# NVIDIA/CUDALibrarySamples

Hardware: AMD Instinct MI355X
Metric: contraction GFLOP/s, fp32 einsum abcd,dcbe->ae (higher is better)
Workload: dtype f32

## Files before the change

### cudalibrarysamples_amd/csrc/host/api.cpp

```cpp
#include <algorithm>
#include <cmath>
#include <cstdio>
#include <cstdlib>
#include <cstring>
#include <new>
#include <optional>
#include <sstream>

#include <hip/hip_runtime.h>

#include "internal.hpp"

using namespace ctamd;

static const cutensorComputeDescriptor kCompute[6] = {
    {0, CUTENSOR_COMPUTE_16F}, {1, CUTENSOR_COMPUTE_16BF}, {2, CUTENSOR_COMPUTE_TF32},
    {3, CUTENSOR_COMPUTE_3XTF32}, {4, CUTENSOR_COMPUTE_32F}, {5, CUTENSOR_COMPUTE_64F}};
extern "C" {
const cutensorComputeDescriptor_t CUTENSOR_COMPUTE_DESC_16F    = &kCompute[0];
const cutensorComputeDescriptor_t CUTENSOR_COMPUTE_DESC_16BF   = &kCompute[1];
const cutensorComputeDescriptor_t CUTENSOR_COMPUTE_DESC_TF32   = &kCompute[2];
const cutensorComputeDescriptor_t CUTENSOR_COMPUTE_DESC_3XTF32 = &kCompute[3];
const cutensorComputeDescriptor_t CUTENSOR_COMPUTE_DESC_32F    = &kCompute[4];
const cutensorComputeDescriptor_t CUTENSOR_COMPUTE_DESC_64F    = &kCompute[5];
}

extern "C" int ctamd_h16p_grid_cap;
extern "C" int ctamd_h16p_stagger;
int ctamd_h16p_stagger = [] { const char* e = CTAMD_HOOK_ENV("CUTENSOR_AMD_H16P_STAGGER"); return e ? std::atoi(e) : -1; }();
int ctamd_h16p_grid_cap = [] { const char* e = CTAMD_HOOK_ENV("CUTENSOR_AMD_H16P_GRID"); const int v = e ? std::atoi(e) : 0; return v > 0 ? v : 0; }();

namespace {

std::atomic<uint64_t> g_launchCounts[5];
std::atomic<int> g_lastH16Kernel{-1};

bool valid_compute(cutensorComputeDescriptor_t c) { return c >= &kCompute[0] && c <= &kCompute[5]; }

int log_level() {
    static int lvl = [] {
        const char* e = std::getenv("CUTENSOR_LOG_LEVEL");
        return e ? std::atoi(e) : 0;
    }();
    return lvl;
}
#define CT_LOG(...) do { if (log_level() > 0) { std::fprintf(stderr, "[cutensor-amd] " __VA_ARGS__); std::fputc('\n', stderr); } } while (0)

bool supported_dtype(hipDataType t) {
    return t == HIP_R_32F || t == HIP_R_64F || t == HIP_R_16F || t == HIP_R_16BF || t == HIP_C_32F || t == HIP_C_64F;
}

hipDataType scalar_type_for(hipDataType data, const cutensorComputeDescriptor* c) {
    if (data == HIP_C_32F || data == HIP_C_64F) return data;
    if (data == HIP_R_64F || (c && c->id == 5)) return HIP_R_64F;
    return HIP_R_32F;
}

cutensorStatus_t fill_use(TensorUse& u, const cutensorTensorDescriptor_t d, const int32_t* modes,
                          cutensorOperator_t op) {
    if (d == nullptr) return CUTENSOR_STATUS_INVALID_VALUE;
    if (d->numModes > 0 && modes == nullptr) return CUTENSOR_STATUS_INVALID_VALUE;
    u.desc = *d;
    u.modes.assign(modes, modes + d->numModes);
    u.op = op;
    u.present = true;
    return CUTENSOR_STATUS_SUCCESS;
}

double num_elements(const cutensorTensorDescriptor& d) {
    double n = 1.0;
    for (int64_t e : d.extent) n *= (double)e;
    return n;
}

std::string problem_key(const cutensorOperationDescriptor& op) {
    std::ostringstream ss;
    ss << (int)op.kind << ':' << (int)op.A.desc.dtype << ':' << (op.compute ? op.compute->id : -1);
    if ((op.D.present && op.D.desc.dtype != op.A.desc.dtype) || (op.C.present && op.C.desc.dtype != op.A.desc.dtype))
        ss << ":d" << (int)op.D.desc.dtype << ":c" << (op.C.present ? (int)op.C.desc.dtype : -1);
    auto put = [&](const TensorUse& u) {
        ss << '|';
        if (!u.present) return;
        for (size_t i = 0; i < u.modes.size(); ++i)
            ss << u.modes[i] << ',' << u.desc.extent[i] << ',' << u.desc.stride[i] << ';';
        ss << 'a' << u.desc.alignment;
    };
    put(op.A); put(op.B); put(op.C); put(op.D);
    return ss.str();
}

bool build_memo_key(const cutensorOperationDescriptor& op, const cutensorPlanPreference& pr, uint64_t wsLimit, PlanMemoKey& k) {
    if (op.kind != OpKind::Contraction && op.kind != OpKind::Reduction && op.kind != OpKind::Permutation &&
        op.kind != OpKind::ElementwiseBinary) return false;
    if (!op.padLeft.empty() || !op.padRight.empty()) return false;
    const TensorUse* u[4] = {&op.A, &op.B, &op.C, &op.D};
    size_t total = 0;
    for (const TensorUse* t : u) if (t->present) total += t->modes.size();
    if (total > (size_t)PlanMemoKey::kMaxModes) return false;
    k.wsLimit = wsLimit;
    k.algo = (int32_t)pr.algo; k.kernelRank = pr.kernelRank; k.autotune = (int32_t)pr.autotune;
    k.incrementalCount = pr.autotune == CUTENSOR_AUTOTUNE_MODE_INCREMENTAL ? pr.incrementalCount : 0;
    k.operandsStreamed = (uint8_t)(pr.operandsStreamed != 0);
    k.kind = (uint8_t)op.kind; k.dtype = (uint8_t)op.A.desc.dtype; k.compute = (uint8_t)(op.compute ? op.compute->id : 255);
    k.scalarType = (uint8_t)op.scalarType;
    k.dtypeD = op.D.present ? (uint8_t)op.D.desc.dtype : (uint8_t)255; k.dtypeC = op.C.present ? (uint8_t)op.C.desc.dtype : (uint8_t)255;
    k.op[0] = (uint8_t)op.A.op; k.op[1] = (uint8_t)op.B.op; k.op[2] = (uint8_t)op.C.op; k.op[3] = (uint8_t)op.opReduce;
    k.present = 0;
    uint32_t w = 0;
    for (int i = 0; i < 4; ++i) {
        const TensorUse& t = *u[i];
        k.n[i] = 0; k.alignment[i] = 0;
        if (!t.present) continue;
        k.present |= (uint8_t)(1u << i);
        const size_t n = t.modes.size();
        k.n[i] = (uint8_t)n; k.alignment[i] = t.desc.alignment;
        for (size_t j = 0; j < n; ++j) k.data[w++] = t.modes[j];
        std::memcpy(&k.data[w], t.desc.extent.data(), n * sizeof(int64_t)); w += (uint32_t)n;
        std::memcpy(&k.data[w], t.desc.stride.data(), n * sizeof(int64_t)); w += (uint32_t)n;
    }
    k.used = w;
    return true;
}

}

uint64_t PlanMemoKey::hash() const {
    auto mix = [](uint64_t h, uint64_t v) { h ^= v; h *= 0x9E3779B97F4A7C15ull; return h ^ (h >> 29); };
    uint64_t h = 0xCBF29CE484222325ull;
    const size_t headWords = offsetof(PlanMemoKey, data) / 8;
    const uint64_t* p = reinterpret_cast<const uint64_t*>(this);
    for (size_t i = 0; i < headWords; ++i) h = mix(h, p[i]);
    for (uint32_t i = 0; i < used; ++i) h = mix(h, (uint64_t)data[i]);
    return h;
}
bool PlanMemoKey::operator==(const PlanMemoKey& o) const {
    return used == o.used && std::memcmp(this, &o, offsetof(PlanMemoKey, data)) == 0 &&
           std::memcmp(data, o.data, (size_t)used * sizeof(int64_t)) == 0;
}

namespace {

bool plan_env_override() {
    return CTAMD_HOOK_ENV("CUTENSOR_AMD_FORCE") || CTAMD_HOOK_ENV("CUTENSOR_AMD_XCD_BALANCE") || CTAMD_HOOK_ENV("CUTENSOR_AMD_FUSED_FOLD") ||
           CTAMD_HOOK_ENV("CUTENSOR_AMD_H16_TRANSPOSE_T1") || CTAMD_HOOK_ENV("CUTENSOR_AMD_NT") || CTAMD_HOOK_ENV("CUTENSOR_AMD_H16_WAVES") || CTAMD_HOOK_ENV("CUTENSOR_AMD_H16_SPLITK") ||
           CTAMD_HOOK_ENV("CUTENSOR_AMD_KORDER") || CTAMD_HOOK_ENV("CUTENSOR_AMD_ABLATION") || CTAMD_HOOK_ENV("CUTENSOR_AMD_PEEL") || CTAMD_HOOK_ENV("CUTENSOR_AMD_GEN") ||
           CTAMD_HOOK_ENV("CUTENSOR_AMD_REPACK") || CTAMD_HOOK_ENV("CUTENSOR_AMD_EW_ANY") || CTAMD_HOOK_ENV("CUTENSOR_AMD_F32X") ||
           CTAMD_HOOK_ENV("CUTENSOR_AMD_F64X");
}

double scalar_as_double(const void* s, hipDataType t) {
    if (s == nullptr) return 0.0;
    return (t == HIP_R_64F || t == HIP_C_64F) ? *static_cast<const double*>(s) : (double)*static_cast<const float*>(s);
}
double scalar_imag(const void* s, hipDataType t) {
    if (s == nullptr) return 0.0;
    if (t == HIP_C_64F) return static_cast<const double*>(s)[1];
    if (t == HIP_C_32F) return (double)static_cast<const float*>(s)[1];
    return 0.0;
}

bool misaligned(const void* p, uint32_t a) { return a > 1 && (reinterpret_cast<uintptr_t>(p) % a) != 0; }

constexpr uint64_t align256(uint64_t bytes) { return (bytes + 255) & ~255ull; }
struct TwoStepLayout {
    const uint64_t offB, offW;
    TwoStepLayout(uint64_t bytesA, uint64_t bytesB) : offB(align256(bytesA)), offW(offB + align256(bytesB)) {}
};

bool names_candidate(const cutensorPlanPreference& pr) { return (int)pr.algo >= 0 || pr.kernelRank > 0; }
bool names_candidate_or_tunes(const cutensorPlanPreference& pr) { return names_candidate(pr) || pr.algo == CUTENSOR_ALGO_DEFAULT_PATIENT || pr.autotune == CUTENSOR_AUTOTUNE_MODE_INCREMENTAL; }

const GettKernelInfo* kernel_table(int family, int* count) { return family == 2 ? gett_gen_kernels(count) : family == 1 ? gett_h16_kernels(count) : gett_f32_kernels(count); }
const GettKernelInfo* kernel_info(int family, int kernel) {
    int n = 0;
    const GettKernelInfo* tab = kernel_table(family, &n);
    return (kernel >= 0 && kernel < n) ? &tab[kernel] : nullptr;
}

}

static void resolve_pending_measurements(cutensorHandle* handle) {
    std::vector<cutensorHandle::PendingMeasurement> todo;
    {
        std::lock_guard<std::mutex> g(handle->mtx);
        todo.swap(handle->pending);
        handle->pendingCount.store(0, std::memory_order_relaxed);
    }
    for (auto& m : todo) {
        float ms = 0.f;
        const bool ok = hipEventSynchronize(m.e1) == hipSuccess && hipEventElapsedTime(&ms, m.e0, m.e1) == hipSuccess;
        (void)hipEventDestroy(m.e0);
        (void)hipEventDestroy(m.e1);
        if (!ok) { (void)hipGetLastError(); continue; }
        std::lock_guard<std::mutex> g(handle->mtx);
        cutensorHandle::TuneState& t = handle->tuning[m.key];
        CT_LOG("incremental autotune: kernel %d splitK %u -> %.3f us (best so far %.3f us)", m.kernel, m.splitK, ms * 1e3, t.bestMs * 1e3);
        if (ms < t.bestMs) {
            t.bestMs = ms; t.bestKernel = m.kernel; t.bestSplitK = m.splitK;
            if (handle->planCache.count(m.key) || handle->planCache.size() < handle->planCacheCapacity) {
                handle->planCache[m.key] = PlanCacheEntry{m.key, m.kernel, m.splitK};
                handle->planMemo.clear();
            }
        }
    }
}

static bool plan_is_plain(const cutensorPlan& pl) { return pl.tuneKey.empty() && pl.wideTab.empty() && !pl.bsp; }
static bool plan_has_sub_plans(const cutensorPlan& pl) { return pl.sub1 || pl.sub2 || pl.loneA || pl.loneB; }
static cutensorPlan* clone_plan(const cutensorPlan& src) { return new (std::nothrow) cutensorPlan(src); }
static bool plan_is_prototype(const cutensorPlan& pl) {
    if (!plan_is_plain(pl)) return false;
    if (!plan_has_sub_plans(pl)) return true;
    if (pl.kind != OpKind::Contraction || (pl.planKind != PlanKind::LoneReduce && pl.planKind != PlanKind::Repack) || pl.sub2 || !pl.sub1) return false;
    for (const SubPlan* q : {&pl.sub1, &pl.loneA, &pl.loneB})
        if (*q && (!plan_is_plain(**q) || plan_has_sub_plans(**q))) return false;
    return true;
}
static void memo_insert(cutensorHandle* h, const PlanMemoKey& key, uint64_t hash, const cutensorPlan& pl) {
    if (!plan_is_prototype(pl)) return;
    std::shared_ptr<const cutensorPlan> proto(clone_plan(pl));
    if (!proto) return;
    std::lock_guard<std::mutex> g(h->mtx);
    if (h->planCacheCapacity == 0) return;
    if (h->planMemo.size() >= h->planCacheCapacity && h->planMemo.find(hash) == h->planMemo.end()) {
        auto victim = h->planMemo.begin();
        for (auto it = h->planMemo.begin(); it != h->planMemo.end(); ++it)
            if (it->second.stamp < victim->second.stamp) victim = it;
        h->planMemo.erase(victim);
    }
    PlanMemoEntry& e = h->planMemo[hash];
    e.key = key; e.proto = std::move(proto); e.stamp = ++h->memoClock;
}

static constexpr int64_t kMaxPeelLaunches = 64;
static bool peel_wide_contraction(const cutensorOperationDescriptor& desc, cutensorOperationDescriptor& inner, std::vector<PeelMode>& peel) {
    if (desc.kind != OpKind::Contraction) return false;
    inner = desc;
    peel.clear();
    const bool h16 = dtype_size(desc.A.desc.dtype) == 2;
    int64_t launches = 1;
    auto idx = [](const TensorUse& t, int32_t l) { for (size_t i = 0; i < t.modes.size(); ++i) if (t.modes[i] == l) return (int)i; return -1; };
    for (int round = 0; round < 16; ++round) {
        ContractionView v;
        if (build_contraction_view(inner, v, nullptr) != CUTENSOR_STATUS_SUCCESS) return false;
        if (!v.wide) return !peel.empty();
        const std::vector<CanonMode>* gs[4] = {&v.L, &v.M, &v.N, &v.K};
        int32_t bestLabel = 0;
        int64_t bestExtent = 0;
        for (int g = 0; g < 4; ++g) {
            if ((int)gs[g]->size() <= kMaxGroupModes) continue;
            if (g == 3 && h16) return false;
            for (const CanonMode& m : *gs[g]) {
                const int ia = idx(inner.A, m.label), ib = idx(inner.B, m.label), ic = idx(inner.C, m.label);
                const int64_t e = ia >= 0 ? inner.A.desc.extent[(size_t)ia] : ib >= 0 ? inner.B.desc.extent[(size_t)ib] : ic >= 0 ? inner.C.desc.extent[(size_t)ic] : 0;
                if (e < 2) continue;
                if (bestExtent == 0 || e < bestExtent) { bestLabel = m.label; bestExtent = e; }
            }
        }
        if (bestExtent == 0) return false;
        launches *= bestExtent;
        if (launches > kMaxPeelLaunches) return false;
        const int32_t l = bestLabel;
        PeelMode pm;
        pm.extent = bestExtent;
        const int ia = idx(inner.A, l), ib = idx(inner.B, l), ic = idx(inner.C, l), id = idx(inner.D, l);
        if (ia >= 0) { pm.sA = inner.A.desc.stride[(size_t)ia]; inner.A.desc.extent[(size_t)ia] = 1; }
        if (ib >= 0) { pm.sB = inner.B.desc.stride[(size_t)ib]; inner.B.desc.extent[(size_t)ib] = 1; }
        if (ic >= 0) { pm.sC = inner.C.desc.stride[(size_t)ic]; inner.C.desc.extent[(size_t)ic] = 1; }
        if (id >= 0) { pm.sD = inner.D.desc.stride[(size_t)id]; inner.D.desc.extent[(size_t)id] = 1; }
        pm.contracted = (ic < 0);
        peel.push_back(pm);
    }
    return false;
}
struct TwoStepSplit {
    cutensorOperationDescriptor inner, stepA, stepB;
    bool hasA = false, hasB = false;
    uint64_t bytesA = 0, bytesB = 0;
    int64_t summedA = 1, summedB = 1;
};
struct PackedTemporary {
    TensorUse use;
    int64_t   elems = 1;
    explicit PackedTemporary(const TensorUse& X) { use.present = true; use.op = X.op; use.desc.dtype = X.desc.dtype; use.desc.alignment = 128; }
    void push(int32_t label, int64_t extent) {
        use.modes.push_back(label); use.desc.extent.push_back(extent); use.desc.stride.push_back(elems);
        use.desc.numModes += 1; elems *= extent;
    }
    uint64_t bytes() const { return (uint64_t)elems * dtype_size(use.desc.dtype); }
};
static bool split_lone_modes(const cutensorOperationDescriptor& desc, TwoStepSplit& out) {
    auto has = [](const std::vector<int32_t>& v, int32_t l) { return std::find(v.begin(), v.end(), l) != v.end(); };
    auto reduce_operand = [&](const TensorUse& X, const TensorUse& other, cutensorOperationDescriptor& red, TensorUse& kept, uint64_t& bytes,
                              int64_t& summed) {
        bool lone = false;
        for (size_t i = 0; i < X.modes.size(); ++i)
            if (X.desc.extent[i] != 1 && !has(other.modes, X.modes[i]) && !has(desc.C.modes, X.modes[i])) lone = true;
        if (!lone) return false;
        PackedTemporary t(X);
        summed = 1;
// ... 1386 lines not shown
            if (clone == nullptr) return CUTENSOR_STATUS_ALLOC_FAILED;
            handle->memoHits.fetch_add(1, std::memory_order_relaxed);
            *plan = clone;
            return CUTENSOR_STATUS_SUCCESS;
        }
        handle->memoMisses.fetch_add(1, std::memory_order_relaxed);
    }
    std::unique_ptr<cutensorPlan> pl(new (std::nothrow) cutensorPlan());
    if (pl == nullptr) return CUTENSOR_STATUS_ALLOC_FAILED;
    pl->kind = desc->kind;
    pl->dtype = desc->A.desc.dtype;
    pl->scalarType = desc->scalarType;
    pl->alignA = desc->A.desc.alignment;
    pl->alignB = desc->B.present ? desc->B.desc.alignment : 0;
    pl->alignC = desc->C.present ? desc->C.desc.alignment : 0;
    pl->alignD = desc->D.desc.alignment;
    pl->accumulate64 = desc->compute && desc->compute->id == 5;
    const cutensorStatus_t st = build_plan(PlanRequest{handle, *desc, pref, pr, workspaceSizeLimit}, *pl);
    if (st != CUTENSOR_STATUS_SUCCESS) return st;
    if (memoable) memo_insert(handle, mkey, mhash, *pl);
    *plan = pl.release();
    return CUTENSOR_STATUS_SUCCESS;
} CTAMD_API_CATCH


cutensorStatus_t cutensorDestroyPlan(cutensorPlan_t plan) try {
    delete plan;
    return CUTENSOR_STATUS_SUCCESS;
} CTAMD_API_CATCH

cutensorStatus_t cutensorPlanGetAttribute(const cutensorHandle_t handle, const cutensorPlan_t plan,
                                          cutensorPlanAttribute_t attr, void* buf, size_t sizeInBytes) try {
    if (handle == nullptr) return CUTENSOR_STATUS_NOT_INITIALIZED;
    if (plan == nullptr || buf == nullptr) return CUTENSOR_STATUS_INVALID_VALUE;
    if (attr == CUTENSOR_PLAN_REQUIRED_WORKSPACE && sizeInBytes == sizeof(uint64_t)) {
        *static_cast<uint64_t*>(buf) = plan->requiredWorkspace;
        return CUTENSOR_STATUS_SUCCESS;
    }
    return CUTENSOR_STATUS_INVALID_VALUE;
} CTAMD_API_CATCH

struct CallScalars { double a, b, aIm, bIm; };
static const void* scalar_constant(hipDataType scalarType, bool one) {
    static const float f[2][2] = {{0.f, 0.f}, {1.f, 0.f}};
    static const double d[2][2] = {{0.0, 0.0}, {1.0, 0.0}};
    return (scalarType == HIP_R_64F || scalarType == HIP_C_64F) ? static_cast<const void*>(d[one]) : static_cast<const void*>(f[one]);
}
static cutensorStatus_t run_two_step(const cutensorHandle_t handle, const cutensorPlan& plan, const void* alpha, const void* A, const void* B,
                                     const void* beta, const void* C, void* D, void* workspace, uint64_t workspaceSize, cudaStream_t stream) {
    if (!plan.sub1) return CUTENSOR_STATUS_INVALID_VALUE;
    const TwoStepLayout lay(plan.loneBytesA, plan.loneBytesB);
    char* ws = static_cast<char*>(workspace);
    const void* one = scalar_constant(plan.scalarType, true);
    const void* zero = scalar_constant(plan.scalarType, false);
    const float scaleA = std::ldexp(1.f, -plan.loneShiftA), scaleB = std::ldexp(1.f, -plan.loneShiftB);
    const bool scaled = plan.loneShiftA + plan.loneShiftB > 0;
    const float alphaScaled = scaled ? *static_cast<const float*>(alpha) * std::ldexp(1.f, plan.loneShiftA + plan.loneShiftB) : 0.f;
    auto first_step = [&](const SubPlan& step, const float& scale, const void* X, char* T) {
        return plan.planKind == PlanKind::Repack ? cutensorPermute(handle, step.get(), one, X, T, stream)
                                                 : cutensorReduce(handle, step.get(), scaled ? &scale : one, X, zero, T, T, ws + lay.offW, workspaceSize - lay.offW, stream);
    };
    cutensorStatus_t st = CUTENSOR_STATUS_SUCCESS;
    if (plan.loneA) { st = first_step(plan.loneA, scaleA, A, ws); A = ws; }
    if (st == CUTENSOR_STATUS_SUCCESS && plan.loneB) { st = first_step(plan.loneB, scaleB, B, ws + lay.offB); B = ws + lay.offB; }
    if (st != CUTENSOR_STATUS_SUCCESS) return st;
    return cutensorContract(handle, plan.sub1.get(), scaled ? &alphaScaled : alpha, A, B, beta, C, D, ws + lay.offW, workspaceSize - lay.offW, stream);
}
static cutensorStatus_t run_peeled(const cutensorHandle_t handle, const cutensorPlan& plan, const void* alpha, const void* A, const void* B,
                                   const void* beta, const void* C, void* D, void* workspace, uint64_t workspaceSize, cudaStream_t stream) {
    if (!plan.sub1) return CUTENSOR_STATUS_INVALID_VALUE;
    const int64_t es = (int64_t)dtype_size(plan.dtype);
    const void* one = scalar_constant(plan.scalarType, true);
    const size_t n = plan.peel.size();
    std::vector<int64_t> digit(n, 0);
    for (;;) {
        int64_t oA = 0, oB = 0, oC = 0, oD = 0;
        bool first = true;
        for (size_t i = 0; i < n; ++i) {
            const PeelMode& pm = plan.peel[i];
            oA += digit[i] * pm.sA; oB += digit[i] * pm.sB; oC += digit[i] * pm.sC; oD += digit[i] * pm.sD;
            if (pm.contracted && digit[i] != 0) first = false;
        }
        char* d = static_cast<char*>(D) + oD * es;
        const char* c = first ? (C ? static_cast<const char*>(C) + oC * es : nullptr) : d;
        const cutensorStatus_t st = cutensorContract(handle, (!first && plan.sub2) ? plan.sub2.get() : plan.sub1.get(), alpha, static_cast<const char*>(A) + oA * es,
                                                     static_cast<const char*>(B) + oB * es, first ? beta : one, c, d, workspace, workspaceSize, stream);
        if (st != CUTENSOR_STATUS_SUCCESS) return st;
        size_t i = 0;
        for (; i < n; ++i) {
            if (++digit[i] < plan.peel[i].extent) break;
            digit[i] = 0;
        }
        if (i == n) return CUTENSOR_STATUS_SUCCESS;
    }
}
struct ProfiledLaunch {
    cutensorHandle* handle;
    hipStream_t stream;
    hipEvent_t e0 = nullptr, e1 = nullptr;
    ProfiledLaunch(cutensorHandle* h, hipStream_t s) : handle(h), stream(s) {
        if (h->prof.enabled.load(std::memory_order_relaxed) && hipEventCreate(&e0) == hipSuccess && hipEventCreate(&e1) == hipSuccess)
            (void)hipEventRecord(e0, stream);
    }
    void end() {
        if (!e0 || !e1) return;
        (void)hipEventRecord(e1, stream);
        std::lock_guard<std::mutex> g(handle->prof.mtx);
        handle->prof.events.emplace_back(e0, e1);
    }
};
static bool mode_table_on_device(const cutensorHandle_t handle, cutensorPlan& plan) {
    if (plan.wideDev) return true;
    std::lock_guard<std::mutex> g(handle->mtx);
    if (!plan.wideDev) plan.wideDev = upload_mode_table(plan.wideTab);
    return plan.wideDev != nullptr;
}
static hipError_t launch_mode_table(const cutensorPlan& plan, const GettParams& p, const CallScalars& s, hipStream_t stream) {
    WideParams w = plan.wide;
    w.modes = plan.wideDev.get();
    w.A = p.A; w.B = p.B; w.C = p.C; w.D = p.D;
    w.alpha = p.alpha; w.beta = p.beta; w.alpha64 = s.a; w.beta64 = s.b;
    w.alphaIm = s.aIm; w.betaIm = s.bIm;
    g_launchCounts[1].fetch_add(1, std::memory_order_relaxed);
    return launch_gett_wide(w, (int)plan.dtype, plan.accumulate64, stream);
}
static hipError_t launch_strip_plan(const ContractionChoice& c, const GettKernelInfo& ki, const GettKernelInfo& ks, const GettParams& p, hipStream_t stream) {
    const uint32_t mInt = c.mInt, nInt = c.nInt, Mt = p.gM.total, Nt = p.gN.total, Lt = p.gL.total;
    GettParams q = p;
    q.tilesM = mInt / (uint32_t)ki.bm; q.tilesN = nInt / (uint32_t)ki.bn;
    q.nBlocks = q.tilesM * q.tilesN * Lt;
    const hipError_t err = ki.launch(q, stream);
    GettParams s2 = p;
    s2.mOrg = mInt; s2.nOrg = 0;
    s2.tilesM = (Mt - mInt + (uint32_t)ks.bm - 1u) / (uint32_t)ks.bm; s2.tilesN = (Nt + (uint32_t)ks.bn - 1u) / (uint32_t)ks.bn;
    s2.mOrg2 = 0; s2.nOrg2 = nInt;
    s2.tilesM2 = (mInt + (uint32_t)ks.bm - 1u) / (uint32_t)ks.bm; s2.tilesN2 = (Nt - nInt + (uint32_t)ks.bn - 1u) / (uint32_t)ks.bn;
    if (s2.tilesM * s2.tilesN == 0u) {
        s2.mOrg = s2.mOrg2; s2.nOrg = s2.nOrg2; s2.tilesM = s2.tilesM2; s2.tilesN = s2.tilesN2;
        s2.tilesM2 = s2.tilesN2 = 0;
    }
    s2.nBlocks = (s2.tilesM * s2.tilesN + s2.tilesM2 * s2.tilesN2) * Lt;
    return (err == hipSuccess && s2.nBlocks > 0u) ? ks.launch(s2, stream) : err;
}
static hipError_t launch_tiled(const cutensorHandle_t handle, const cutensorPlan& plan, GettParams& p, const CallScalars& s, void* workspace, hipStream_t stream) {
    const ContractionChoice& c = plan.choice;
    int count = 0;
    const GettKernelInfo* tab = kernel_table(c.family, &count);
    g_launchCounts[2 + c.family].fetch_add(1, std::memory_order_relaxed);
    p.partial = (c.splitK > 1) ? static_cast<float*>(workspace) : nullptr;
    int launchKernel = c.kernel;
    if (c.family == 0) {
        static const int policy = [] { const char* e = CTAMD_HOOK_ENV("CUTENSOR_AMD_PARTIAL_STORE"); return e ? (e[0] == 'p' ? 1 : e[0] == 'n' ? 2 : e[0] == 's' ? 3 : 0) : 0; }();
        p.partialPolicy = policy;
        if (plan.fusedFold) {
            uint32_t slot;
            {
                std::lock_guard<std::mutex> g(handle->mtx);
                slot = handle->syncNext++ % cutensorHandle::kSyncSlots;
            }
            p.sync = handle->syncPool + (size_t)slot * 16;
        }
    } else if (c.family == 1) {
        static const bool persistentForced = CTAMD_HOOK_ENV("CUTENSOR_AMD_H16_WAVES") != nullptr && h16_waves_variant() == H16_W4P;
        if (tab[launchKernel].variant == H16_W4P && s.b != 0.0 && p.cStrideN[0] != 1 && !persistentForced)
            launchKernel = h16_entry(H16_W4X, launchKernel - H16_W4P);
        g_lastH16Kernel.store(launchKernel, std::memory_order_relaxed);
    }
    ProfiledLaunch prof(handle, stream);
    hipError_t err = (c.family == 1 && c.stripKernel >= 0 && c.stripKernel < count) ? launch_strip_plan(c, tab[launchKernel], tab[c.stripKernel], p, stream)
                                                                                    : tab[launchKernel].launch(p, stream);
    prof.end();
    if (err != hipSuccess || c.splitK <= 1 || (c.family == 0 && (plan.fusedFold || handle->skipFold.load(std::memory_order_relaxed)))) return err;
    SplitKReduceParams r = plan.skr;
    r.partial = static_cast<float*>(workspace);
    r.C = p.C; r.D = p.D; r.alpha = p.alpha; r.beta = p.beta;
    r.alpha64 = s.a; r.beta64 = s.b; r.alphaIm = s.aIm; r.betaIm = s.bIm; r.conjC = p.conjC;
    return launch_splitk_fold(c.family, tab[c.kernel], r, stream);
}

cutensorStatus_t cutensorContract(const cutensorHandle_t handle, const cutensorPlan_t plan, const void* alpha,
                                  const void* A, const void* B, const void* beta, const void* C, void* D,
                                  void* workspace, uint64_t workspaceSize, cudaStream_t stream) try {
    if (handle == nullptr) return CUTENSOR_STATUS_NOT_INITIALIZED;
    if (plan == nullptr || plan->kind != OpKind::Contraction) return CUTENSOR_STATUS_INVALID_VALUE;
    if (alpha == nullptr || beta == nullptr || A == nullptr || B == nullptr || D == nullptr) return CUTENSOR_STATUS_INVALID_VALUE;
    const CallScalars s{scalar_as_double(alpha, plan->scalarType), scalar_as_double(beta, plan->scalarType), scalar_imag(alpha, plan->scalarType),
                        scalar_imag(beta, plan->scalarType)};
    const bool betaZero = (s.b == 0.0 && s.bIm == 0.0);
    if (!betaZero && C == nullptr) return CUTENSOR_STATUS_INVALID_VALUE;
    if (misaligned(A, plan->alignA) || misaligned(B, plan->alignB) || misaligned(D, plan->alignD) ||
        (!betaZero && misaligned(C, plan->alignC)))
        return CUTENSOR_STATUS_INVALID_VALUE;
    if (plan->requiredWorkspace > 0 && (workspace == nullptr || workspaceSize < plan->requiredWorkspace))
        return CUTENSOR_STATUS_INSUFFICIENT_WORKSPACE;
    switch (plan->planKind) {
        case PlanKind::LoneReduce:
        case PlanKind::Repack: return run_two_step(handle, *plan, alpha, A, B, beta, C, D, workspace, workspaceSize, stream);
        case PlanKind::Peeled: return run_peeled(handle, *plan, alpha, A, B, beta, C, D, workspace, workspaceSize, stream);
        case PlanKind::ModeTable:
            if (!mode_table_on_device(handle, *plan)) return CUTENSOR_STATUS_ALLOC_FAILED;
            break;
        default: break;
    }
    GettParams p = plan->gett;
    p.A = plan->view.swapped ? B : A;
    p.B = plan->view.swapped ? A : B;
    p.C = (!betaZero) ? C : D;
    p.D = D;
    p.alpha = (float)s.a; p.beta = (float)s.b;
    p.alpha64 = s.a; p.beta64 = s.b;
    p.alphaIm = s.aIm; p.betaIm = s.bIm;
    p.endA += (unsigned long long)(uintptr_t)p.A;
    p.endB += (unsigned long long)(uintptr_t)p.B;
    p.timing = handle->timingBuffer.load(std::memory_order_relaxed);
    hipEvent_t t0 = nullptr, t1 = nullptr;
    if (!plan->tuneKey.empty() && plan->trial.timed.load(std::memory_order_relaxed) < cutensorPlan::kTrialTimedRuns &&
        plan->trial.timed.fetch_add(1, std::memory_order_relaxed) < cutensorPlan::kTrialTimedRuns) {
        if (hipEventCreate(&t0) != hipSuccess || hipEventCreate(&t1) != hipSuccess) {
            (void)hipGetLastError();
            if (t0) (void)hipEventDestroy(t0);
            t0 = t1 = nullptr;
        } else {
            (void)hipEventRecord(t0, stream);
        }
    }
    hipError_t err;
    if (plan->planKind == PlanKind::ModeTable) err = launch_mode_table(*plan, p, s, stream);
    else if (plan->planKind == PlanKind::Tiled) err = launch_tiled(handle, *plan, p, s, workspace, stream);
    else {
        g_launchCounts[0].fetch_add(1, std::memory_order_relaxed);
        p.partial = nullptr;
        err = launch_gett_simple(p, (int)plan->dtype, plan->accumulate64, stream);
    }
    if (t0 != nullptr) {
        if (err == hipSuccess && hipEventRecord(t1, stream) == hipSuccess) {
            std::lock_guard<std::mutex> g(handle->mtx);
            handle->pending.push_back(cutensorHandle::PendingMeasurement{plan->tuneKey, plan->choice.kernel, plan->choice.splitK, t0, t1});
            handle->pendingCount.store((int)handle->pending.size(), std::memory_order_relaxed);
        } else {
            (void)hipEventDestroy(t0);
            (void)hipEventDestroy(t1);
        }
    }
    if (err != hipSuccess) { CT_LOG("cutensorContract: %s", hipGetErrorString(err)); return CUTENSOR_STATUS_EXECUTION_FAILED; }
    return CUTENSOR_STATUS_SUCCESS;
} CTAMD_API_CATCH

static hipError_t run_elementwise(const EwPlan& ew, hipDataType dtype, double a, const void* A, double g,
                                  const void* C, void* D, hipStream_t stream, const void* E = nullptr, double d = 0.0,
                                  double aIm = 0.0, double gIm = 0.0) {
    Ew2DParams p = ew.p;
    p.A = A;
    p.C = (ew.usesC && (g != 0.0 || gIm != 0.0 || (p.opAC != 0 && p.opAC != CUTENSOR_OP_ADD))) ? C : nullptr;
    p.D = D;
    p.E = E;
    p.alpha = (float)a; p.gamma = (float)g; p.alpha64 = a; p.gamma64 = g;
    p.alphaIm = aIm; p.gammaIm = gIm;
    p.delta = (float)d; p.delta64 = d;
    const int variant = (ew.variant == EW_BLOCK && p.unA != 0) ? ew.blockFrom : ew.variant;
    if (ew.converts()) return launch_elementwise_convert(p, variant, (int)ew.dtypeA, (int)ew.dtypeD, stream);
    return launch_elementwise(p, variant, (int)dtype, stream);
}

cutensorStatus_t cutensorReduce(const cutensorHandle_t handle, const cutensorPlan_t plan, const void* alpha,
                                const void* A, const void* beta, const void* C, void* D, void* workspace,
                                uint64_t workspaceSize, cudaStream_t stream) try {
    if (handle == nullptr) return CUTENSOR_STATUS_NOT_INITIALIZED;
    if (plan == nullptr || plan->kind != OpKind::Reduction) return CUTENSOR_STATUS_INVALID_VALUE;
    if (alpha == nullptr || beta == nullptr || A == nullptr || D == nullptr) return CUTENSOR_STATUS_INVALID_VALUE;
    const double a = scalar_as_double(alpha, plan->scalarType), b = scalar_as_double(beta, plan->scalarType);
    const double aIm = scalar_imag(alpha, plan->scalarType), bIm = scalar_imag(beta, plan->scalarType);
    const bool betaSet = b != 0.0 || bIm != 0.0;
    if (betaSet && C == nullptr) return CUTENSOR_STATUS_INVALID_VALUE;
    if (misaligned(A, plan->alignA) || misaligned(D, plan->alignD) || (betaSet && misaligned(C, plan->alignC)))
        return CUTENSOR_STATUS_INVALID_VALUE;
    hipError_t err;
    if (plan->red.isPermutation) {
        err = run_elementwise(plan->red.perm, plan->dtype, a, A, b, C, D, stream, nullptr, 0.0, aIm, bIm);
    } else {
        if (plan->requiredWorkspace > 0 && (workspace == nullptr || workspaceSize < plan->requiredWorkspace))
            return CUTENSOR_STATUS_INSUFFICIENT_WORKSPACE;
        ReduceParams p = plan->red.p;
        p.A = A; p.C = betaSet ? C : D; p.D = D;
        p.alpha = (float)a; p.beta = (float)b; p.alpha64 = a; p.beta64 = b;
        p.alphaIm = aIm; p.betaIm = bIm;
        p.partial = (p.splitR > 1) ? workspace : nullptr;
        const bool acc64 = plan->accumulate64 || plan->dtype == HIP_R_64F;
        err = launch_reduce(p, plan->red.variant, (int)plan->dtype, acc64, stream);
        if (err == hipSuccess && p.splitR > 1) err = launch_reduce_finalize(p, (int)plan->dtype, acc64, stream);
    }
    if (err != hipSuccess) { CT_LOG("cutensorReduce: %s", hipGetErrorString(err)); return CUTENSOR_STATUS_EXECUTION_FAILED; }
    return CUTENSOR_STATUS_SUCCESS;
} CTAMD_API_CATCH

cutensorStatus_t cutensorPermute(const cutensorHandle_t handle, const cutensorPlan_t plan, const void* alpha,
                                 const void* A, void* B, const cudaStream_t stream) try {
    if (handle == nullptr) return CUTENSOR_STATUS_NOT_INITIALIZED;
    if (plan == nullptr || plan->kind != OpKind::Permutation) return CUTENSOR_STATUS_INVALID_VALUE;
    if (alpha == nullptr || A == nullptr || B == nullptr) return CUTENSOR_STATUS_INVALID_VALUE;
    if (misaligned(A, plan->alignA) || misaligned(B, plan->alignD)) return CUTENSOR_STATUS_INVALID_VALUE;
    const double a = scalar_as_double(alpha, plan->scalarType);
    hipError_t err = hipSuccess;
    void* out = B;
    if (plan->padFillElems != 0) {
        err = launch_fill(B, plan->padFillElems, (int)plan->ew.dtypeD, plan->padValue, stream);
        out = static_cast<char*>(B) + plan->padOffsetElems * (int64_t)dtype_size(plan->ew.dtypeD);
    }
    if (err == hipSuccess) err = run_elementwise(plan->ew, plan->dtype, a, A, 0.0, nullptr, out, stream, nullptr, 0.0, scalar_imag(alpha, plan->scalarType));
    if (err != hipSuccess) { CT_LOG("cutensorPermute: %s", hipGetErrorString(err)); return CUTENSOR_STATUS_EXECUTION_FAILED; }
    return CUTENSOR_STATUS_SUCCESS;
} CTAMD_API_CATCH

cutensorStatus_t cutensorElementwiseBinaryExecute(const cutensorHandle_t handle, const cutensorPlan_t plan,
                                                  const void* alpha, const void* A, const void* gamma,
                                                  const void* C, void* D, cudaStream_t stream) try {
    if (handle == nullptr) return CUTENSOR_STATUS_NOT_INITIALIZED;
    if (plan == nullptr || plan->kind != OpKind::ElementwiseBinary) return CUTENSOR_STATUS_INVALID_VALUE;
    if (alpha == nullptr || gamma == nullptr || A == nullptr || C == nullptr || D == nullptr) return CUTENSOR_STATUS_INVALID_VALUE;
    if (misaligned(A, plan->alignA) || misaligned(C, plan->alignC) || misaligned(D, plan->alignD)) return CUTENSOR_STATUS_INVALID_VALUE;
    const double a = scalar_as_double(alpha, plan->scalarType), g = scalar_as_double(gamma, plan->scalarType);
    hipError_t err = run_elementwise(plan->ew, plan->dtype, a, A, g, C, D, stream, nullptr, 0.0, scalar_imag(alpha, plan->scalarType),
                                     scalar_imag(gamma, plan->scalarType));
    if (err != hipSuccess) return CUTENSOR_STATUS_EXECUTION_FAILED;
    return CUTENSOR_STATUS_SUCCESS;
} CTAMD_API_CATCH

cutensorStatus_t cutensorElementwiseTrinaryExecute(const cutensorHandle_t handle, const cutensorPlan_t plan,
                                                   const void* alpha, const void* A, const void* beta, const void* B,
                                                   const void* gamma, const void* C, void* D, cudaStream_t stream) try {
    if (handle == nullptr) return CUTENSOR_STATUS_NOT_INITIALIZED;
    if (plan == nullptr || plan->kind != OpKind::ElementwiseTrinary) return CUTENSOR_STATUS_INVALID_VALUE;
    if (alpha == nullptr || beta == nullptr || gamma == nullptr || A == nullptr || B == nullptr || C == nullptr || D == nullptr)
        return CUTENSOR_STATUS_INVALID_VALUE;
    if (misaligned(A, plan->alignA) || misaligned(B, plan->alignB3) || misaligned(C, plan->alignC) || misaligned(D, plan->alignD))
        return CUTENSOR_STATUS_INVALID_VALUE;
    const double a = scalar_as_double(alpha, plan->scalarType), b = scalar_as_double(beta, plan->scalarType),
                 g = scalar_as_double(gamma, plan->scalarType);
    const EwTrinaryPlan& t = plan->ew3;
    hipError_t err = hipSuccess;
    if (t.bothPermuted) {
        Ew2DParams q = t.last.p;
        q.A = A; q.X = B; q.D = D; q.E = nullptr;
        q.C = (t.last.usesC && (g != 0.0 || (q.opAC != 0 && q.opAC != CUTENSOR_OP_ADD))) ? C : nullptr;
        q.alpha = (float)a; q.alpha64 = a; q.xi = (float)b; q.xi64 = b; q.gamma = (float)g; q.gamma64 = g;
        err = launch_elementwise(q, t.last.variant, (int)plan->dtype, stream);
    } else if (t.twoPass) {
        const uintptr_t c = reinterpret_cast<uintptr_t>(C), d = reinterpret_cast<uintptr_t>(D);
        const bool readsC = t.last.usesC && (g != 0.0 || (t.last.p.opAC != 0 && t.last.p.opAC != CUTENSOR_OP_ADD));
        if (readsC && c < d + t.spanD && d < c + t.spanC) {
            if (!t.hasGather) return CUTENSOR_STATUS_NOT_SUPPORTED;
            Ew2DParams q = t.gather.p;
            q.A = A; q.X = B; q.C = C; q.D = D; q.E = nullptr;
            q.alpha = (float)a; q.alpha64 = a; q.xi = (float)b; q.xi64 = b; q.gamma = (float)g; q.gamma64 = g;
            err = launch_elementwise(q, EW_GENERIC, (int)plan->dtype, stream);
        } else {
            err = run_elementwise(t.first, plan->dtype, a, A, 0.0, nullptr, D, stream);
            if (err == hipSuccess) err = run_elementwise(t.last, plan->dtype, b, B, g, C, D, stream, D, 1.0);
        }
    } else if (t.swapAB) {
        err = run_elementwise(t.last, plan->dtype, a, A, g, C, D, stream, B, b);
    } else {
        err = run_elementwise(t.last, plan->dtype, b, B, g, C, D, stream, A, a);
    }
    if (err != hipSuccess) { CT_LOG("cutensorElementwiseTrinaryExecute: %s", hipGetErrorString(err)); return CUTENSOR_STATUS_EXECUTION_FAILED; }
    return CUTENSOR_STATUS_SUCCESS;
} CTAMD_API_CATCH

cutensorStatus_t cutensorContractTrinary(const cutensorHandle_t handle, const cutensorPlan_t plan, const void* alpha,
                                         const void* A, const void* B, const void* C, const void* beta, const void* D, void* E,
                                         void* workspace, uint64_t workspaceSize, cudaStream_t stream) try {
    if (handle == nullptr) return CUTENSOR_STATUS_NOT_INITIALIZED;
    if (plan == nullptr || plan->kind != OpKind::ContractionTrinary || !plan->sub1 || !plan->sub2) return CUTENSOR_STATUS_INVALID_VALUE;
    if (alpha == nullptr || beta == nullptr || A == nullptr || B == nullptr || C == nullptr || E == nullptr) return CUTENSOR_STATUS_INVALID_VALUE;
    if (workspace == nullptr || workspaceSize < plan->requiredWorkspace) return CUTENSOR_STATUS_INSUFFICIENT_WORKSPACE;
    if (misaligned(workspace, 128)) return CUTENSOR_STATUS_INVALID_VALUE;
    const void* in[3] = {A, B, C};
    const void *X = in[plan->triOrder[0]], *Y = in[plan->triOrder[1]], *Z = in[plan->triOrder[2]];
    const uint64_t tOff = align256(plan->tBytes);
    void* T = workspace;
    void* ws = static_cast<char*>(workspace) + tOff;
    const void *one = scalar_constant(plan->scalarType, true), *zero = scalar_constant(plan->scalarType, false);
    cutensorStatus_t st = cutensorContract(handle, plan->sub1.get(), one, X, Y, zero, T, T, ws, workspaceSize - tOff, stream);
    if (st != CUTENSOR_STATUS_SUCCESS) return st;
    return cutensorContract(handle, plan->sub2.get(), alpha, T, Z, beta, D, E, ws, workspaceSize - tOff, stream);
} CTAMD_API_CATCH

cutensorStatus_t cutensorWriteKernelCacheToFile(const cutensorHandle_t handle, const char filename[]) try {
    if (handle == nullptr) return CUTENSOR_STATUS_NOT_INITIALIZED;
    if (filename == nullptr) return CUTENSOR_STATUS_INVALID_VALUE;
    FILE* f = std::fopen(filename, "w");
    if (f == nullptr) return CUTENSOR_STATUS_IO_ERROR;
    std::fprintf(f, "cutensor-amd-kernelcache 1 gfx950 0\n");
    std::fclose(f);
    return CUTENSOR_STATUS_SUCCESS;
} CTAMD_API_CATCH
cutensorStatus_t cutensorReadKernelCacheFromFile(cutensorHandle_t handle, const char filename[]) try {
    if (handle == nullptr) return CUTENSOR_STATUS_NOT_INITIALIZED;
    if (filename == nullptr) return CUTENSOR_STATUS_INVALID_VALUE;
    FILE* f = std::fopen(filename, "r");
    if (f == nullptr) return CUTENSOR_STATUS_IO_ERROR;
    char tag[64] = {0};
    const bool ok = std::fscanf(f, "%63s", tag) == 1 && std::strcmp(tag, "cutensor-amd-kernelcache") == 0;
    std::fclose(f);
    return ok ? CUTENSOR_STATUS_SUCCESS : CUTENSOR_STATUS_IO_ERROR;
} CTAMD_API_CATCH

const char* cutensorGetErrorString(const cutensorStatus_t error) {
    switch (error) {
        case CUTENSOR_STATUS_SUCCESS: return "CUTENSOR_STATUS_SUCCESS";
        case CUTENSOR_STATUS_NOT_INITIALIZED: return "CUTENSOR_STATUS_NOT_INITIALIZED";
        case CUTENSOR_STATUS_ALLOC_FAILED: return "CUTENSOR_STATUS_ALLOC_FAILED";
        case CUTENSOR_STATUS_INVALID_VALUE: return "CUTENSOR_STATUS_INVALID_VALUE";
        case CUTENSOR_STATUS_ARCH_MISMATCH: return "CUTENSOR_STATUS_ARCH_MISMATCH";
        case CUTENSOR_STATUS_MAPPING_ERROR: return "CUTENSOR_STATUS_MAPPING_ERROR";
        case CUTENSOR_STATUS_EXECUTION_FAILED: return "CUTENSOR_STATUS_EXECUTION_FAILED";
        case CUTENSOR_STATUS_INTERNAL_ERROR: return "CUTENSOR_STATUS_INTERNAL_ERROR";
        case CUTENSOR_STATUS_NOT_SUPPORTED: return "CUTENSOR_STATUS_NOT_SUPPORTED";
        case CUTENSOR_STATUS_LICENSE_ERROR: return "CUTENSOR_STATUS_LICENSE_ERROR";
        case CUTENSOR_STATUS_CUBLAS_ERROR: return "CUTENSOR_STATUS_CUBLAS_ERROR";
        case CUTENSOR_STATUS_CUDA_ERROR: return "CUTENSOR_STATUS_CUDA_ERROR";
        case CUTENSOR_STATUS_INSUFFICIENT_WORKSPACE: return "CUTENSOR_STATUS_INSUFFICIENT_WORKSPACE";
        case CUTENSOR_STATUS_INSUFFICIENT_DRIVER: return "CUTENSOR_STATUS_INSUFFICIENT_DRIVER";
        case CUTENSOR_STATUS_IO_ERROR: return "CUTENSOR_STATUS_IO_ERROR";
        default: return "<unknown>";
    }
}

size_t cutensorGetVersion(void) { return CUTENSOR_VERSION; }

int ctamdPlanModeTableGroups(const cutensorPlan_t plan, int32_t* group, int32_t* label, int64_t* extent, int maxOut) try {
    if (plan == nullptr || plan->kind != OpKind::Contraction || plan->planKind != PlanKind::ModeTable) return 0;
    if (plan->view.dtype == HIP_C_32F || plan->view.dtype == HIP_C_64F) return 0;
    int n = 0;
    const std::vector<CanonMode>* gs[4] = {&plan->view.L, &plan->view.M, &plan->view.N, &plan->view.K};
    bool oversized = false;
    for (int g = 0; g < 4; ++g) oversized = oversized || (int)gs[g]->size() > kMaxGroupModes;
    if (!oversized) return 0;
    for (int g = 0; g < 4; ++g)
        for (const CanonMode& m : *gs[g]) {
            if (n < maxOut) { if (group) group[n] = g; if (label) label[n] = m.label; if (extent) extent[n] = m.extent; }
            ++n;
        }
    return n;
} CTAMD_API_CATCH_INT

int ctamdPlanPeelLaunches(const cutensorPlan_t plan) try {
    if (plan == nullptr || plan->kind != OpKind::Contraction || plan->planKind != PlanKind::Peeled) return 0;
    long long n = 1;
    for (const PeelMode& pm : plan->peel) n *= pm.extent;
    return (int)n;
} CTAMD_API_CATCH_INT

int ctamdLastH16Kernel(void) try { return g_lastH16Kernel.load(std::memory_order_relaxed); } CTAMD_API_CATCH_INT

void ctamdLaunchCounts(uint64_t out[5]) try {
    for (int i = 0; i < 5; ++i) out[i] = g_launchCounts[i].load(std::memory_order_relaxed);
} CTAMD_API_CATCH_VOID

void ctamdPlanMemoStats(const cutensorHandle_t handle, uint64_t* hits, uint64_t* misses, uint32_t* entries) try {
    if (handle == nullptr) return;
    if (hits) *hits = handle->memoHits.load(std::memory_order_relaxed);
    if (misses) *misses = handle->memoMisses.load(std::memory_order_relaxed);
    if (entries) { std::lock_guard<std::mutex> g(handle->mtx); *entries = (uint32_t)handle->planMemo.size(); }
} CTAMD_API_CATCH_VOID
static int describe_inner(const cutensorPlan& plan, char* buf, size_t len, int n);
static int describe_unary(char* buf, size_t len, int n, int32_t a, int32_t b, int32_t c) {
    if ((a == 0 && b == 0 && c == 0) || n <= 0 || (size_t)n >= len || buf[n - 1] != '}') return n;
    auto code = [](int32_t u) { return u == 0 ? (int)CUTENSOR_OP_IDENTITY : (int)u; };
    return n - 1 + std::snprintf(buf + n - 1, len - (size_t)n + 1, ",\"unary\":[%d,%d,%d]}", code(a), code(b), code(c));
}
int ctamdDescribePlan(const cutensorPlan_t plan, char* buf, size_t len) try {
    if (plan == nullptr || buf == nullptr || len == 0) return -1;
    int n = 0;
    if (plan->kind == OpKind::BlockSparseContraction) return blocksparse_describe(*plan, buf, len);
    if (plan->kind == OpKind::ContractionTrinary)
        return std::snprintf(buf, len, "{\"op\":\"contraction_trinary\",\"intermediate_bytes\":%llu,\"workspace\":%llu}",
                             (unsigned long long)plan->tBytes, (unsigned long long)plan->requiredWorkspace);
    if (plan->kind == OpKind::Contraction && plan->planKind == PlanKind::Peeled && plan->sub1) {
        long long launches = 1;
        int contracted = 0;
        for (const PeelMode& pm : plan->peel) { launches *= pm.extent; contracted += pm.contracted ? 1 : 0; }
        n = std::snprintf(buf, len, "{\"peeled_modes\":%zu,\"peeled_contracted\":%d,\"peel_launches\":%lld,", plan->peel.size(), contracted, launches);
        return describe_inner(*plan, buf, len, n);
    }
    if (plan->kind == OpKind::Contraction && (plan->planKind == PlanKind::LoneReduce || plan->planKind == PlanKind::Repack) && plan->sub1) {
        const bool rep = plan->planKind == PlanKind::Repack, hasA = (bool)plan->loneA, hasB = (bool)plan->loneB;
        n = std::snprintf(buf, len, "{\"lone_reduce_A\":%d,\"lone_reduce_B\":%d,\"repack_A\":%d,\"repack_B\":%d,\"lone_bytes\":%llu,",
                          (hasA && !rep) ? 1 : 0, (hasB && !rep) ? 1 : 0, (hasA && rep) ? 1 : 0, (hasB && rep) ? 1 : 0,
                          (unsigned long long)(plan->loneBytesA + plan->loneBytesB));
        return describe_inner(*plan, buf, len, n);
    }
    if (plan->kind == OpKind::Contraction) {
        static const int kindCode[] = {0, -1, -2, -3, -4, -4};
        int count = 0;
        const GettKernelInfo* tab = kernel_table(plan->choice.family, &count);
        const int k = plan->planKind == PlanKind::Tiled ? plan->choice.kernel : -1;
        n = std::snprintf(buf, len,
                          "{\"op\":\"contraction\",\"family\":%d,\"L\":%llu,\"M\":%llu,\"N\":%llu,\"K\":%llu,\"swapped\":%d,\"layA\":%d,\"layB\":%d,"
                          "\"kernel\":%d,\"bm\":%d,\"bn\":%d,\"bk\":%d,\"wm\":%d,\"wn\":%d,\"wk\":%d,\"pf\":%d,\"abl\":%d,\"splitK\":%u,\"kPerSlice\":%u,"
                          "\"blocks\":%u,\"workspace\":%llu,\"model_us\":%.2f,\"fusedFold\":%d,\"xcdTiles\":\"%016llx\",\"kname\":\"%s\"",
                          plan->choice.family, (unsigned long long)plan->view.totL, (unsigned long long)plan->view.totM,
                          (unsigned long long)plan->view.totN, (unsigned long long)plan->view.totK, (int)plan->view.swapped,
                          plan->view.layA, plan->view.layB, k >= 0 ? k : kindCode[(int)plan->planKind], k >= 0 ? tab[k].bm : 16, k >= 0 ? tab[k].bn : 16,
                          k >= 0 ? tab[k].bk : 16, k >= 0 ? tab[k].wm : 1, k >= 0 ? tab[k].wn : 1, k >= 0 ? tab[k].wk : 1,
                          k >= 0 ? tab[k].pf : 0, k >= 0 ? tab[k].ablation : 0,
                          plan->gett.splitK, plan->gett.kPerSlice, plan->gett.nBlocks,
                          (unsigned long long)plan->requiredWorkspace, plan->choice.estimateUs, (int)plan->fusedFold,
                          (unsigned long long)plan->gett.xcdTiles,
                          k >= 0 ? tab[k].name : plan->planKind == PlanKind::ModeTable ? "gett_wide_kernel" : "gett_simple_kernel");
        if (n > 0 && (size_t)n < len && k >= 0)
            n += std::snprintf(buf + n, len - n, ",\"nt\":%d", tab[k].nt);
        if (n > 0 && (size_t)n < len && plan->choice.family == 2 && k >= 0)
            n += std::snprintf(buf + n, len - n, ",\"orientA\":%d,\"orientB\":%d,\"vec\":%d,\"elem\":%d", tab[k].layA, tab[k].layB, tab[k].vec, tab[k].elem);
        if (n > 0 && (size_t)n < len && plan->choice.family == 1 && k >= 0)
            n += std::snprintf(buf + n, len - n, ",\"rag\":%d,\"strips\":%d,\"mInt\":%u,\"nInt\":%u",
                               (plan->gett.gK.total % 64u != 0u || (plan->gett.ragged & 1u)) ? 1 : 0, plan->choice.stripKernel >= 0 ? 1 : 0,
                               plan->choice.mInt, plan->choice.nInt);
        if (n > 0 && (size_t)n < len) n += std::snprintf(buf + n, len - n, ",\"Kdigits\":[");
        for (size_t i = 0; i < plan->view.K.size() && n > 0 && (size_t)n < len; ++i)
            n += std::snprintf(buf + n, len - n, "%s[%lld,%lld,%lld]", i ? "," : "", (long long)plan->view.K[i].extent,
                               (long long)plan->view.K[i].sA, (long long)plan->view.K[i].sB);
        if (n > 0 && (size_t)n < len) n += std::snprintf(buf + n, len - n, "]}");
    } else if (plan->kind == OpKind::Reduction && !plan->red.isPermutation) {
        n = std::snprintf(buf, len, "{\"op\":\"reduction\",\"variant\":%d,\"kept\":%u,\"red\":%u,\"splitR\":%u,\"redPerSplit\":%u,\"rowAny\":%u,\"workspace\":%llu}",
                          plan->red.variant, plan->red.p.kept.total, plan->red.p.red.total, plan->red.p.splitR, plan->red.p.redPerSplit,
                          plan->red.p.rowAny, (unsigned long long)plan->requiredWorkspace);
        n = describe_unary(buf, len, n, plan->red.p.unA, 0, plan->red.p.unC);
    } else if (plan->kind == OpKind::ElementwiseTrinary) {
        const EwTrinaryPlan& t = plan->ew3;
        n = std::snprintf(buf, len, "{\"op\":\"elementwise\",\"form\":\"trinary\",\"passes\":%d,\"bothPermuted\":%d,\"swapAB\":%d,\"variant\":%d,\"variant_first\":%d,"
                          "\"variant_inplace\":%d,\"E0\":%u,\"E1\":%u,\"rest\":%u,\"blocks\":%u,\"tile0\":%u}",
                          t.twoPass ? 2 : 1, (int)t.bothPermuted, (int)t.swapAB, t.last.variant, t.twoPass ? t.first.variant : -1,
                          t.hasGather ? t.gather.variant : -1, t.last.p.E0, t.last.p.E1, t.last.p.rest.total, t.last.p.nBlocks, t.last.p.tile0);
        const Ew2DParams& q = t.last.p;
        const int32_t uA = t.bothPermuted ? q.unA : t.twoPass ? t.first.p.unA : t.swapAB ? q.unA : q.unE;
        const int32_t uB = t.bothPermuted ? q.unX : t.twoPass ? q.unA : t.swapAB ? q.unE : q.unA;
        n = describe_unary(buf, len, n, uA, uB, q.unC);
    } else {
        const EwPlan& e = (plan->kind == OpKind::Reduction) ? plan->red.perm : plan->ew;
        n = std::snprintf(buf, len, "{\"op\":\"elementwise\",\"variant\":%d,\"E0\":%u,\"E1\":%u,\"rest\":%u,\"blocks\":%u,\"tile0\":%u,\"order\":%u}",
                          e.variant, e.p.E0, e.p.E1, e.p.rest.total, e.p.nBlocks, e.p.tile0, e.p.order);
        n = describe_unary(buf, len, n, e.p.unA, 0, e.p.unC);
        if (e.converts() && n > 1 && (size_t)n < len && buf[n - 1] == '}')
            n = n - 1 + std::snprintf(buf + n - 1, len - (size_t)n + 1, ",\"convert\":[%d,%d]}", (int)e.dtypeA, (int)e.dtypeD);
    }
    return n;
} CTAMD_API_CATCH_INT
static int describe_inner(const cutensorPlan& plan, char* buf, size_t len, int n) {
    if (n < 0 || (size_t)n >= len) return -1;
    const int m = ctamdDescribePlan(plan.sub1.get(), buf + n - 1, len - (size_t)n + 1);
    if (m < 0) return -1;
    buf[n - 1] = ',';
    return n - 1 + m;
}

void ctamdSetTimingBuffer(cutensorHandle_t handle, void* deviceBuffer) try {
    if (handle != nullptr) handle->timingBuffer.store(static_cast<unsigned long long*>(deviceBuffer), std::memory_order_relaxed);
} CTAMD_API_CATCH_VOID

void ctamdSetSplitKFold(cutensorHandle_t handle, int enabled) try {
    if (handle != nullptr) handle->skipFold.store(enabled == 0, std::memory_order_relaxed);
} CTAMD_API_CATCH_VOID

void ctamdProfileBegin(cutensorHandle_t handle) try {
    if (handle == nullptr) return;
    std::lock_guard<std::mutex> g(handle->prof.mtx);
    handle->prof.events.clear();
    handle->prof.enabled.store(true, std::memory_order_relaxed);
} CTAMD_API_CATCH_VOID
int ctamdProfileEnd(cutensorHandle_t handle, float* meanMs, float* minMs) try {
    if (handle == nullptr) return 0;
    std::lock_guard<std::mutex> g(handle->prof.mtx);
    handle->prof.enabled.store(false, std::memory_order_relaxed);
    double sum = 0.0;
    float mn = 1e30f;
    int n = 0;
    for (auto& ev : handle->prof.events) {
        float t = 0.f;
        if (hipEventSynchronize(ev.second) == hipSuccess && hipEventElapsedTime(&t, ev.first, ev.second) == hipSuccess) {
            sum += t;
            mn = std::min(mn, t);
            ++n;
        }
        (void)hipEventDestroy(ev.first);
        (void)hipEventDestroy(ev.second);
    }
    handle->prof.events.clear();
    if (meanMs) *meanMs = n ? (float)(sum / n) : 0.f;
    if (minMs) *minMs = n ? mn : 0.f;
    return n;
} CTAMD_API_CATCH_INT

int ctamdTestHooksBuilt(void) try { return CTAMD_HOOKS_BUILT; } CTAMD_API_CATCH_INT

int ctamdKernelCount(void) try {
    int count = 0;
    (void)kernel_table(0, &count);
    return count;
} CTAMD_API_CATCH_INT
int ctamdKernelIsAblation(int i) try {
    const GettKernelInfo* k = kernel_info(0, i);
    return (k != nullptr && k->ablation) ? 1 : 0;
} CTAMD_API_CATCH_INT

int ctamdCountCandidates(const cutensorHandle_t handle, const cutensorOperationDescriptor_t desc, uint64_t wsLimit) try {
    if (handle == nullptr || desc == nullptr || desc->kind != OpKind::Contraction) return -1;
    ContractionView v;
    if (build_contraction_view(*desc, v, nullptr) != CUTENSOR_STATUS_SUCCESS) return -1;
    if (v.dtype != HIP_R_32F || v.wide) return 0;
    return (int)rank_contraction_choices(v, wsLimit, handle->numCUs).size();
// ... 4 lines not shown
```

### cudalibrarysamples_amd/csrc/host/plan_contraction.cpp

```cpp
#include <algorithm>
#include <cmath>
#include <cstdlib>
#include <cstring>

#include "internal.hpp"

namespace ctamd {

FastDiv make_fastdiv(uint32_t d) {
    FastDiv f{};
    f.d = d;
    if (d < 2) {
        f.magic = 0;
        f.shift = 0;
        return f;
    }
    uint32_t s = 0;
    while ((1ull << s) < d) ++s;
    const uint64_t m = ((1ull << (31 + s)) / d) + 1;
    f.magic = (uint32_t)m;
    f.shift = s - 1;
    return f;
}

// ... 167 lines not shown
    if (v.totL > lim || v.totM > lim || v.totN > lim || (int)v.L.size() > kMaxGroupModes || (int)v.M.size() > kMaxGroupModes ||
        (int)v.N.size() > kMaxGroupModes || (int)v.K.size() > kMaxGroupModes) {
        if (v.L.size() + v.M.size() + v.N.size() + v.K.size() > 128) return fail(CUTENSOR_STATUS_NOT_SUPPORTED, "more than 128 unfusable modes");
        v.wide = true;
        v.layA = v.layB = LAY_S;
        return CUTENSOR_STATUS_SUCCESS;
    }
    v.alignA = v.swapped ? op.B.desc.alignment : op.A.desc.alignment;
    v.alignB = v.swapped ? op.A.desc.alignment : op.B.desc.alignment;
    v.alignD = op.D.desc.alignment;
    if (v.dtype == HIP_C_32F || v.dtype == HIP_C_64F) {
        v.layA = v.layB = LAY_S;
        return CUTENSOR_STATUS_SUCCESS;
    }

    const int64_t vec = (dtype_size(v.dtype) == 2) ? 8 : 4;
    auto all_mult4_except = [vec](const std::vector<const std::vector<CanonMode>*>& groups, bool slotA,
                                  const CanonMode* except) {
        for (auto* g : groups)
            for (const CanonMode& m : *g) {
                if (&m == except) continue;
                const int64_t s = slotA ? m.sA : m.sB;
                if (s % vec != 0) return false;
            }
        return true;
    };
    const uint32_t alignA = v.swapped ? op.B.desc.alignment : op.A.desc.alignment;
    const uint32_t alignB = v.swapped ? op.A.desc.alignment : op.B.desc.alignment;
    auto pick16 = [&](bool slotA, const std::vector<CanonMode>& freeG) {
        const std::vector<CanonMode>* groups[3] = {&freeG, &v.K, &v.L};
        for (const std::vector<CanonMode>* g : groups)
            for (const CanonMode& m : *g)
                if ((slotA ? m.sA : m.sB) < 0) return (int)LAY_S;
        if (!v.K.empty()) {
            const CanonMode& k0 = v.K.front();
            if ((slotA ? k0.sA : k0.sB) == 1 && (k0.extent % 8 == 0 || v.K.size() == 1)) return (int)LAY_K;
        }
        if (!freeG.empty()) {
            const CanonMode& f0 = freeG.front();
            if ((slotA ? f0.sA : f0.sB) == 1 && (f0.extent % 8 == 0 || freeG.size() == 1)) return (int)LAY_F;
        }
        return (int)LAY_S;
    };
    if (dtype_size(v.dtype) == 2) {
        v.layA = pick16(true, v.M);
        v.layB = pick16(false, v.N);
        return CUTENSOR_STATUS_SUCCESS;
    }
    auto pick = [&](bool slotA, const std::vector<CanonMode>& freeG, uint32_t align) {
        if (align % 16 != 0) return (int)LAY_S;
        std::vector<const std::vector<CanonMode>*> groups = {&freeG, &v.K, &v.L};
        if (!v.K.empty()) {
            const CanonMode& k0 = v.K.front();
            const int64_t s = slotA ? k0.sA : k0.sB;
            if (s == 1 && k0.extent % vec == 0 && all_mult4_except(groups, slotA, &k0)) return (int)LAY_K;
        }
        if (!freeG.empty()) {
            const CanonMode& f0 = freeG.front();
            const int64_t s = slotA ? f0.sA : f0.sB;
            if (s == 1 && f0.extent % vec == 0 && all_mult4_except(groups, slotA, &f0)) return (int)LAY_F;
        }
        return (int)LAY_S;
    };
    v.layA = pick(true, v.M, alignA);
    v.layB = pick(false, v.N, alignB);
    v.lanesA = v.layA != LAY_S;
    v.lanesB = v.layB != LAY_S;
    auto pick32 = [&](bool slotA, const std::vector<CanonMode>& freeG) {
        const std::vector<CanonMode>* groups[3] = {&freeG, &v.K, &v.L};
        for (const std::vector<CanonMode>* g : groups)
            for (const CanonMode& m : *g)
                if ((slotA ? m.sA : m.sB) < 0) return (int)LAY_S;
        if (!v.K.empty()) {
            const CanonMode& k0 = v.K.front();
            if ((slotA ? k0.sA : k0.sB) == 1 && (k0.extent % 4 == 0 || v.K.size() == 1)) return (int)LAY_K;
        }
        if (!freeG.empty()) {
            const CanonMode& f0 = freeG.front();
            if ((slotA ? f0.sA : f0.sB) == 1 && (f0.extent % 4 == 0 || freeG.size() == 1)) return (int)LAY_F;
        }
        return (int)LAY_S;
    };
    if (v.dtype == HIP_R_32F) {
        if (!v.lanesA) v.layA = pick32(true, v.M);
        if (!v.lanesB) v.layB = pick32(false, v.N);
    }
    return CUTENSOR_STATUS_SUCCESS;
}

static bool f32_needs_rag(const ContractionView& v) {
    return v.totK % 32 != 0 || !v.lanesA || !v.lanesB;
}

static double tile_efficiency(const GettKernelInfo& k) {
    const int area = k.bm * k.bn;
    const int ringDepth = k.pf;
    if (k.fragPartials) return area >= 96 * 96 ? (ringDepth == 4 ? 0.93 : 0.92) : 0.75;
    if (area >= 128 * 128) return 0.85;
    if (area >= 96 * 96) return 0.80;
    if (area >= 64 * 64) return 0.65;
    if (area >= 48 * 48) return 0.70;
    return 0.45;
}

std::vector<ContractionChoice> rank_contraction_choices(const ContractionView& v, uint64_t wsLimit,
                                                        int numCUs, bool operandsStreamed) {
    std::vector<ContractionChoice> out;
    int count = 0;
    const GettKernelInfo* tab = gett_f32_kernels(&count);
    const double clk = 2.4e9, flopPerClkCU = 256.0;
    const double hbm = 6.0e12, l2bw = 20.0e12;
    const double M = (double)v.totM, N = (double)v.totN, K = (double)v.totK, L = (double)v.totL;

    const bool withAblations = CTAMD_HOOK_ENV("CUTENSOR_AMD_ABLATION") != nullptr;
    auto span_bytes = [&](bool slotA) {
        uint64_t n = 1;
        for (const std::vector<CanonMode>* g : {slotA ? &v.M : &v.N, &v.K})
            for (const CanonMode& m : *g) n += (uint64_t)(m.extent - 1) * (uint64_t)std::llabs(slotA ? m.sA : m.sB);
        return n * 4ull;
    };
    const bool fits32 = span_bytes(true) < (1ull << 32) - (1ull << 20) && span_bytes(false) < (1ull << 32) - (1ull << 20);
    auto full_span_bytes = [&](bool slotA) {
        uint64_t n = span_bytes(slotA) / 4ull;
        for (const CanonMode& m : v.L) n += (uint64_t)(m.extent - 1) * (uint64_t)std::llabs(slotA ? m.sA : m.sB);
        return n * 4ull;
    };
    const bool fits31 = full_span_bytes(true) < (1ull << 31) - (1ull << 20) && full_span_bytes(false) < (1ull << 31) - (1ull << 20);
    const bool needRag = f32_needs_rag(v);
    for (int i = 0; i < count; ++i) {
        const GettKernelInfo& k = tab[i];
        if (k.ablation && !withAblations) continue;
        if (k.fragPartials && !fits32) continue;
        const bool rag = k.fragPartials && needRag;
        const int effA = (k.fragPartials || v.lanesA) ? v.layA : (int)LAY_S, effB = (k.fragPartials || v.lanesB) ? v.layB : (int)LAY_S;
        const bool okA = (k.layA == effA) || (k.layA == LAY_S);
        const bool okB = (k.layB == effB) || (k.layB == LAY_S);
        if (!okA || !okB) continue;
        if ((k.layA == LAY_S) != (k.layB == LAY_S)) continue;
        if (k.layA == LAY_S && v.lanesA && v.lanesB) continue;
        if (rag && (!fits31 || k.nt || k.ablation || (v.K.size() > 1 && v.totK % k.bk != 0))) continue;
        if (k.kfast && !(rag && v.K.size() == 1) && (v.K.empty() || (v.K.front().extent % k.bk) != 0)) continue;

        const uint64_t tilesM = (v.totM + k.bm - 1) / k.bm, tilesN = (v.totN + k.bn - 1) / k.bn;
        const uint64_t tiles = tilesM * tilesN * v.totL;
        static const bool ntAnySize = CTAMD_HOOK_ENV("CUTENSOR_AMD_NT") != nullptr;
        if (k.nt && !(tilesM == 1 && tilesN == 1 && (ntAnySize || operandsStreamed || 4.0 * L * (M * K + N * K) > 1.4 * 256.0 * 1024.0 * 1024.0))) continue;
        const uint64_t kTiles = (v.totK + k.bk - 1) / k.bk;
        std::vector<uint32_t> splits = {1};
        for (uint32_t s = 2; s <= 1024; s *= 2) {
            if (kTiles / s < 4) break;
            if (tiles * s > (uint64_t)numCUs * 16) break;
            splits.push_back(s);
        }
        for (uint32_t s : splits) {
            ContractionChoice c;
            c.kernel = i;
            if (k.fragPartials && v.totK % k.bk != 0 && !rag) continue;
            const uint64_t tilesPerSlice = (kTiles + s - 1) / s;
            c.kPerSlice = (uint32_t)(tilesPerSlice * k.bk);
            c.splitK = (uint32_t)((v.totK + c.kPerSlice - 1) / c.kPerSlice);
            if (c.splitK < 1) c.splitK = 1;
            if (c.splitK != s && s != 1) continue;
            if (k.fragPartials)
                c.workspace = (c.splitK > 1) ? (uint64_t)c.splitK * tiles * k.bm * k.bn * 4ull : 0ull;
            else
                c.workspace = (c.splitK > 1) ? (uint64_t)c.splitK * v.totL * v.totM * v.totN * 4ull : 0ull;
            if (c.workspace > wsLimit) continue;

            const double blocks = (double)tiles * c.splitK;
            const double wgPerCU = k.fragPartials ? 1.0 : 2.0;
            const double slots = numCUs * wgPerCU;
            const double rounds = std::ceil(blocks / slots);
            const double flopsBlock = 2.0 * k.bm * k.bn * (double)c.kPerSlice;
            const double tBlock = flopsBlock / (flopPerClkCU * clk * tile_efficiency(k) / wgPerCU);
            const double occupancyFill = std::min(1.0, blocks / slots);
            double tCompute = rounds * tBlock * (occupancyFill < 1.0 && blocks < numCUs ? 0.5 : 1.0);
            if (blocks <= numCUs) tCompute = flopsBlock / (flopPerClkCU * clk * tile_efficiency(k));
            const double bytesA = 4.0 * L * (double)tilesM * k.bm * K * (double)tilesN;
            const double bytesB = 4.0 * L * (double)tilesN * k.bn * K * (double)tilesM;
            const double bytesUnique = 4.0 * L * (M * K + N * K + M * N);
            const double bytesPartial = (c.splitK > 1) ? 2.0 * (double)c.workspace : 0.0;
            const double tMem = std::max((bytesA + bytesB) / l2bw, (bytesUnique + bytesPartial) / hbm);
            const double tFold = (c.splitK > 1 && c.splitK < 32 && k.fragPartials) ? (double)c.workspace / 5.0e12 * (32.0 / c.splitK - 1.0) : 0.0;
            const double ldsBytes = k.fragPartials ? (double)k.pf * (k.bm + k.bn) * k.bk * 4.0 : 0.0;
            const double overlap = (!k.fragPartials || ldsBytes <= 80.0 * 1024.0) ? 2.0 : 1.0;
            const double roundsEff = std::ceil(blocks / (numCUs * overlap));
            const double shortK = std::max(0.0, 1.0 - (double)tilesPerSlice / 64.0);
            const double tRound = (roundsEff > 1.0) ? (roundsEff - 1.0) * (2.0e-6 + 0.34e-6 * (double)(k.bm * k.bn) / 1024.0) * shortK : 0.0;
            const double tFix = ((c.splitK > 1) ? 3.0e-6 + tFold : 0.0) + tRound;
            c.estimateUs = (std::max(tCompute, tMem) + tFix + 2.0e-6) * 1e6;
            const int ringDepth = k.pf;
            if (k.fragPartials && ringDepth == 3) c.estimateUs *= 0.999;
            if (k.nt) c.estimateUs *= 0.96;
            out.push_back(c);
        }
    }
    std::stable_sort(out.begin(), out.end(),
                     [](const ContractionChoice& a, const ContractionChoice& b) { return a.estimateUs < b.estimateUs; });
    return out;
}

static bool h16_sweep_ragged(const ContractionView& v) {
    if (v.K.size() < 2 || v.K.front().extent % 64 == 0) return false;
    if (v.layA == LAY_K || v.layB == LAY_K) { if (v.K.front().extent % 8 != 0) return false; }
    if (v.layA == LAY_F && (v.M.empty() || v.M.front().extent % 8 != 0)) return false;
    if (v.layB == LAY_F && (v.N.empty() || v.N.front().extent % 8 != 0)) return false;
    return true;
}
static double h16_sweep_fill(const ContractionView& v) {
    const int64_t e0 = v.K.front().extent;
    return (double)e0 / (64.0 * (double)((e0 + 63) / 64));
}
static uint64_t h16_k_tiles(const ContractionView& v) {
    if (h16_sweep_ragged(v)) return (uint64_t)((v.K.front().extent + 63) / 64) * (v.totK / (uint64_t)v.K.front().extent);
    return (v.totK + 63) / 64;
}

static bool h16_needs_rag(const ContractionView& v) {
    if (v.totK % 64 != 0 || h16_sweep_ragged(v)) return true;
    if (v.layA == LAY_F && !v.M.empty() && v.M.front().extent % 8 != 0) return true;
    if (v.layB == LAY_F && !v.N.empty() && v.N.front().extent % 8 != 0) return true;
    return false;
}

int h16_waves_variant() {
    static const struct { const char* prefix; H16Variant variant; } names[] = {
        {"4s", H16_W4S}, {"4r", H16_W4R}, {"4v", H16_W4V}, {"4x", H16_W4X}, {"4p", H16_W4P}, {"4q", H16_W4Q}, {"8m", H16_W8M},
        {"4m4", H16_W4M4}, {"4m", H16_W4M}, {"4", H16_W4}, {"s", H16_S}, {"8", H16_W8}, {"p", H16_W8}};
    static const int variant = [] {
        const char* e = CTAMD_HOOK_ENV("CUTENSOR_AMD_H16_WAVES");
        for (const auto& n : names)
            if (e && std::strncmp(e, n.prefix, std::strlen(n.prefix)) == 0) return (int)n.variant;
        return (int)H16_W4X;
    }();
    return variant;
}

bool pick_h16_choice(const ContractionView& v, uint64_t wsLimit, int numCUs, ContractionChoice& c) {
    if (v.dtype != HIP_R_16BF && v.dtype != HIP_R_16F) return false;
    if ((v.layA != LAY_K && v.layA != LAY_F) || (v.layB != LAY_K && v.layB != LAY_F)) return false;
    if (v.K.empty()) return false;
    const bool sweep = h16_sweep_ragged(v);
    if (!sweep && ((v.totK % 64 != 0) ? (v.K.size() != 1) : (v.K.front().extent % 64 != 0))) return false;
    if (sweep && h16_k_tiles(v) >= (1ull << 30)) return false;
    if (sweep && h16_sweep_fill(v) < 0.45 && !CTAMD_HOOK_ENV("CUTENSOR_AMD_H16_WAVES")) return false;
    const bool ragged = h16_needs_rag(v);
    auto tile_span_bytes = [&](bool slotA) {
        uint64_t n = 1;
        for (const CanonMode& m : (slotA ? v.M : v.N))
            n += (uint64_t)(std::min<int64_t>(m.extent, 256) - 1) * (uint64_t)std::llabs(slotA ? m.sA : m.sB);
        n += 64ull * (uint64_t)std::llabs(slotA ? v.K.front().sA : v.K.front().sB);
        return n * 2ull;
    };
    if (tile_span_bytes(true) >= (1ull << 31) || tile_span_bytes(false) >= (1ull << 31)) return false;
    for (const std::vector<CanonMode>* g : {&v.M, &v.N, &v.K})
        for (const CanonMode& m : *g)
            if (m.sA < 0 || m.sB < 0) return false;
    int count = 0;
    const GettKernelInfo* tab = gett_h16_kernels(&count);
    c = ContractionChoice{};
    c.family = 1;
    c.kernel = (v.dtype == HIP_R_16BF ? 0 : 4) + (v.layA == LAY_F ? 2 : 0) + (v.layB == LAY_F ? 1 : 0);
    const int variant = h16_waves_variant();
    const bool forced = CTAMD_HOOK_ENV("CUTENSOR_AMD_H16_WAVES") != nullptr;
    const int layoutIdx = c.kernel;
    const uint64_t kTiles = h16_k_tiles(v);
    const uint64_t perSliceBytes = v.totL * v.totM * v.totN * 4ull;
    auto tiles_of = [&](int var) {
        const GettKernelInfo& k = tab[layoutIdx + var];
        return std::ceil((double)v.totM / k.bm) * std::ceil((double)v.totN / k.bn) * (double)v.totL;
    };
    auto slots_of = [&](int var) { return (double)numCUs * ((var == H16_W4M || var == H16_W4Q) ? 2.0 : 1.0); };
    auto auto_split = [&](int var) -> uint64_t {
        const double tiles = tiles_of(var), slots = slots_of(var);
        uint64_t split = 1;
        if (tiles * 2.0 <= slots && kTiles >= 8) {
            split = std::min<uint64_t>((uint64_t)(slots / tiles), kTiles / 4);
            while (split > 1 && split * perSliceBytes > wsLimit) --split;
            if (split < 2) split = 1;
        }
        return split;
    };
    auto model_tiles_us = [&](int var, double tiles, uint64_t split) {
        const double wgs = tiles * (double)split, slots = slots_of(var);
        const double kt = std::ceil((double)kTiles / (double)split);
        double fix, per;
        if (var == H16_W4M4) { fix = 4.5; per = 0.46; }
        else if (var == H16_W4Q) { fix = wgs <= (double)numCUs ? 4.4 : 4.6; per = wgs <= (double)numCUs ? 0.223 : 0.31; }
        else if (var == H16_W4M) { fix = 5.0; per = wgs <= (double)numCUs ? 0.68 : 0.92; }
        else { fix = 10.0; per = 1.0; }
        double t = std::ceil(wgs / slots) * (fix + kt * per);
        if (var == H16_W4P) { const double ke = kt + (std::fmod(kt, 2.0) != 0.0 ? 1.0 : 0.0); t = 10.5 + ke * per + (std::ceil(wgs / slots) - 1.0) * (4.5 + ke * per); }
        if (split > 1) t += 3.0 + 2.0 * (double)split * (double)perSliceBytes / 5.0e6;
        return t;
    };
    auto model_us = [&](int var, uint64_t split) { return model_tiles_us(var, tiles_of(var), split); };
    auto strip_us = [&](int cand, uint32_t& mInt, uint32_t& nInt) {
        if (layoutIdx + H16_W4Q >= count || layoutIdx + cand >= count) return 1e30;
        const GettKernelInfo& k = tab[layoutIdx + cand];
        if (k.bm <= 64) return 1e30;
        mInt = (uint32_t)(v.totM / k.bm) * (uint32_t)k.bm;
        nInt = (uint32_t)(v.totN / k.bn) * (uint32_t)k.bn;
        if ((mInt == v.totM && nInt == v.totN) || mInt == 0 || nInt == 0) return 1e30;
        const double tilesInt = (double)(mInt / k.bm) * (double)(nInt / k.bn) * (double)v.totL;
        const double strip = (std::ceil((double)(v.totM - mInt) / 64.0) * std::ceil((double)v.totN / 64.0) +
                              std::ceil((double)mInt / 64.0) * std::ceil((double)(v.totN - nInt) / 64.0)) * (double)v.totL;
// ... 266 lines not shown
```

### cudalibrarysamples_amd/csrc/kernels/gett_f32_stream.hip

```cpp
#include <hip/hip_runtime.h>
#include <stdint.h>
#include <stdlib.h>

#include "params.h"
#include "launch.h"
#include "gett_common.h"

namespace ctamd {

constexpr int kStreamBK = 32;

typedef uint32_t u32x4 __attribute__((ext_vector_type(4)));
#if defined(__HIP_DEVICE_COMPILE__)
typedef __amdgpu_buffer_rsrc_t BufRsrc;
#else
typedef int BufRsrc;
#endif
__device__ __forceinline__ BufRsrc make_rsrc(const float* base, uint32_t records = 0xffffffffu) {
#if defined(__HIP_DEVICE_COMPILE__)
    return __builtin_amdgcn_make_buffer_rsrc(const_cast<float*>(base), 0, (int)records, 0x00020000);
#else
    (void)base; (void)records; return 0;
#endif
}
__device__ __forceinline__ void store_wt_16(f32x4 v, BufRsrc rsrc, uint32_t byteOff) {
#if defined(__HIP_DEVICE_COMPILE__)
    __builtin_amdgcn_raw_buffer_store_b128(__builtin_bit_cast(u32x4, v), rsrc, (int)byteOff, 0,  16);
#else
    (void)v; (void)rsrc; (void)byteOff;
#endif
}
template <int AUX>
__device__ __forceinline__ void store_policy_16(f32x4 v, BufRsrc rsrc, uint32_t byteOff) {
#if defined(__HIP_DEVICE_COMPILE__)
    __builtin_amdgcn_raw_buffer_store_b128(__builtin_bit_cast(u32x4, v), rsrc, (int)byteOff, 0, AUX);
#else
    (void)v; (void)rsrc; (void)byteOff;
#endif
}
template <int AUX = 0>
__device__ __forceinline__ void lds_dma_16(BufRsrc rsrc, uint32_t laneBytes, uint32_t tileBytes, float* dst) {
#if defined(__HIP_DEVICE_COMPILE__)
    __builtin_amdgcn_raw_ptr_buffer_load_lds(rsrc, (__attribute__((address_space(3))) void*)dst, 16, (int)laneBytes, (int)tileBytes, 0, AUX);
#else
    (void)rsrc; (void)laneBytes; (void)tileBytes; (void)dst;
#endif
}

template <int LAY, int ROWS>
struct StreamOperand {
    static_assert(ROWS % 32 == 0, "tile rows must be a multiple of 32");
    static constexpr int PIECES   = ROWS / 8;
    static constexpr int PER_WAVE = PIECES / 4;
    static constexpr int FLOATS   = ROWS * kStreamBK;
    static constexpr int UR       = ROWS / 4;

    uint32_t src[PER_WAVE];

    template <int SLOT_K>
    __device__ __forceinline__ void init(const ModeGroup& gFree, const ModeGroup& gK, uint32_t row0, int wave, int lane) {
        const int64_t strideK0 = gK.stride[SLOT_K][0];
#pragma unroll
        for (int i = 0; i < PER_WAVE; ++i) {
            const int c = wave + 4 * i;
            if constexpr (LAY == LAY_K) {
                const int r = 8 * c + (lane >> 3), p = lane & 7;
                const int u = p ^ ((r >> 1) & 7);
                uint32_t row = row0 + r;
                if (row >= gFree.total) row = gFree.total - 1;
                src[i] = (group_offset32<0>(gFree, row) + 4u * (uint32_t)u) * 4u;
            } else {
                const int g = 64 * c + lane;
                const int kr = g / UR, p = g % UR;
                const int u = (p + 4 * ((kr >> 2) & 1)) % UR;
                uint32_t row = row0 + 4 * u;
                if (row >= gFree.total) row = (gFree.total - 1u) & ~3u;
                src[i] = (group_offset32<0>(gFree, row) + (uint32_t)kr * (uint32_t)strideK0) * 4u;
            }
        }
    }

    template <int AUX = 0>
    __device__ __forceinline__ void issue(BufRsrc X, uint32_t offKBytes, float* stage, int wave) const {
#pragma unroll
        for (int i = 0; i < PER_WAVE; ++i)
            lds_dma_16<AUX>(X, src[i], offKBytes, stage + (wave + 4 * i) * 256);
    }

    __device__ __forceinline__ void mask(int wave, int lane, uint32_t kValid) {
#pragma unroll
        for (int i = 0; i < PER_WAVE; ++i) {
            const int c = wave + 4 * i;
            bool out;
            if constexpr (LAY == LAY_K) {
                const int r = 8 * c + (lane >> 3), p = lane & 7;
                out = 4u * (uint32_t)(p ^ ((r >> 1) & 7)) >= kValid;
            } else {
                out = (uint32_t)((64 * c + lane) / UR) >= kValid;
            }
            src[i] |= out ? 0x80000000u : 0u;
        }
    }
    __device__ __forceinline__ void fix(float* stage, int wave, int lane, uint32_t kValid) const {
        if constexpr (LAY == LAY_K) {
#pragma unroll
            for (int i = 0; i < PER_WAVE; ++i) {
                const int c = wave + 4 * i;
                const int r = 8 * c + (lane >> 3), p = lane & 7;
                const uint32_t k0 = 4u * (uint32_t)(p ^ ((r >> 1) & 7));
                float* at = stage + c * 256 + lane * 4;
                if (k0 < kValid && kValid < k0 + 4u) {
                    const uint32_t v = kValid - k0;
                    if (v <= 1u) at[1] = 0.f;
                    if (v <= 2u) at[2] = 0.f;
                    at[3] = 0.f;
                }
            }
        }
    }

    __device__ static __forceinline__ int frag_base(int rbase, int lane) {
        const int i = lane & 15, q = lane >> 4;
        if constexpr (LAY == LAY_K) {
            const int r = rbase + i;
            return r * 32 + ((q ^ ((r >> 1) & 7)) << 2);
        } else {
            const int n = rbase + i;
            const int p = ((n >> 2) - 4 * (q & 1) + UR) % UR;
            return (4 * q) * ROWS + p * 4 + (n & 3);
        }
    }

    template <int STEP>
    __device__ static __forceinline__ f32x4 fragment(const float* lds, int base) {
        if constexpr (LAY == LAY_K) {
            return *reinterpret_cast<const f32x4*>(lds + (STEP ? (base ^ 16) : base));
        } else {
            f32x4 o;
#pragma unroll
            for (int kk = 0; kk < 4; ++kk) o[kk] = lds[base + (16 * STEP + kk) * ROWS];
            return o;
        }
    }
};

struct KOdometer {
    uint32_t j0, n0, j1, e1, hi;
    uint32_t offA, offB, stepA, stepB, wrapA, wrapB;

    __device__ static __forceinline__ uint32_t sgpr(uint32_t v) { return (uint32_t)__builtin_amdgcn_readfirstlane((int)v); }

    template <bool RAG = false>
    __device__ __forceinline__ void init(const ModeGroup& gK, uint32_t k0) {
        const uint32_t E0 = gK.div[0].d;
        n0 = sgpr((E0 + (RAG ? (uint32_t)kStreamBK - 1u : 0u)) / kStreamBK);
        e1 = sgpr(gK.div[1].d);
        const uint32_t q0 = (E0 < 2) ? k0 : fast_div(k0, gK.div[0]);
        j0 = sgpr((k0 - q0 * E0) / kStreamBK);
        hi = sgpr((e1 < 2) ? q0 : fast_div(q0, gK.div[1]));
        j1 = sgpr(q0 - hi * e1);
        offA = sgpr((uint32_t)group_offset<0>(gK, k0) * 4u);
        offB = sgpr((uint32_t)group_offset<1>(gK, k0) * 4u);
        stepA = sgpr((uint32_t)((int64_t)kStreamBK * gK.stride[0][0]) * 4u);
        stepB = sgpr((uint32_t)((int64_t)kStreamBK * gK.stride[1][0]) * 4u);
        wrapA = sgpr((uint32_t)gK.stride[0][1] * 4u - (n0 - 1) * stepA);
        wrapB = sgpr((uint32_t)gK.stride[1][1] * 4u - (n0 - 1) * stepB);
    }
    __device__ __forceinline__ void advance(const ModeGroup& gK) {
        const bool c0 = (j0 + 1 == n0);
        j0 = c0 ? 0u : j0 + 1;
        offA += c0 ? wrapA : stepA;
        offB += c0 ? wrapB : stepB;
        j1 += c0 ? 1u : 0u;
        if (j1 == e1) {
            j1 = 0;
            hi += 1;
            const uint32_t k = hi * e1 * gK.div[0].d;
            if (k < gK.total) {
                offA = sgpr((uint32_t)group_offset<0>(gK, k) * 4u);
                offB = sgpr((uint32_t)group_offset<1>(gK, k) * 4u);
            }
        }
    }
};

template <int BM_, int BN_, int LA_, int LB_, int S_, int ABL_ = 0, bool RAG_ = false>
struct StreamCfg {
    static constexpr int BM = BM_, BN = BN_, LA = LA_, LB = LB_, S = S_;
    static constexpr bool RAG = RAG_;
    static constexpr int ABL = ABL_;
    static constexpr int TM = BM / 32, TN = BN / 32;
};

#define CTAMD_WAIT_VMCNT(n) asm volatile("s_waitcnt vmcnt(%0)" ::"n"(n) : "memory")

template <class Cfg>
__global__ void __launch_bounds__(512, 2) gett_f32_stream_kernel(const GettParams p) {
    constexpr int BM = Cfg::BM, BN = Cfg::BN, BK = kStreamBK, S = Cfg::S;
    constexpr int TM = Cfg::TM, TN = Cfg::TN;
    using OpA = StreamOperand<Cfg::LA, BM>;
    using OpB = StreamOperand<Cfg::LB, BN>;
    constexpr int STAGE = OpA::FLOATS + OpB::FLOATS;
    constexpr int LOADS = OpA::PER_WAVE + OpB::PER_WAVE;
    static_assert(S >= 3 && S <= 6 && S * STAGE * 4 <= 160 * 1024, "LDS ring must fit 160 KiB");
    static_assert(LOADS * (S - 1) <= 63, "vmcnt is a 6-bit counter");
    __shared__ __attribute__((aligned(16))) float lds[S * STAGE];
    prefetch_kernarg<(int)sizeof(GettParams)>();

    const int tid  = threadIdx.x;
    const int lane = tid & 63;
    const int wave8 = __builtin_amdgcn_readfirstlane(tid >> 6);
    const int wave = wave8 & 3;
    const bool loader = wave8 >= 4;
    unsigned long long* tlog = p.timing ? p.timing + (size_t)blockIdx.x * 16 : nullptr;
    auto lane_now = []() -> int {
#if defined(__HIP_DEVICE_COMPILE__)
        return (int)__builtin_amdgcn_mbcnt_hi(~0u, __builtin_amdgcn_mbcnt_lo(~0u, 0u));
#else
        return 0;
#endif
    };
    auto stamp = [&](int slot) {
        if (tlog != nullptr && wave8 == 0 && lane_now() == 0) tlog[slot] = (slot >= 5 && slot != 7) ? wall_clock64() : __builtin_readcyclecounter();
    };
    stamp(0);
    stamp(5);

    uint32_t id = xcd_remap(blockIdx.x, p.nBlocks);
    const uint32_t mt = id % p.tilesM; id /= p.tilesM;
    const uint32_t nt = id % p.tilesN; id /= p.tilesN;
    const uint32_t slice = id % p.splitK;
    const uint32_t l = id / p.splitK;
    const uint32_t m0 = mt * BM, n0 = nt * BN;
    uint32_t kBegin = slice * p.kPerSlice;
    int nTiles;
    if (p.xcdTiles != 0) {
        const uint32_t q = p.splitK >> 3;
        const uint32_t x = slice / q, j = slice - x * q;
        uint32_t first = 0, mine = 0;
#pragma unroll
        for (uint32_t y = 0; y < 8; ++y) {
            const uint32_t ny = (uint32_t)(p.xcdTiles >> (8 * y)) & 0xffu;
            first += (y < x) ? ny * q : 0u;
            mine = (y == x) ? ny : mine;
        }
        kBegin = (first + j * mine) * BK;
        nTiles = (int)mine;
    } else {
        uint32_t kEnd = kBegin + p.kPerSlice;
        if (kEnd > p.gK.total) kEnd = p.gK.total;
        nTiles = (int)((kEnd - kBegin + (Cfg::RAG ? (uint32_t)BK - 1u : 0u)) / BK);
    }

    if (loader) {
        const float* baseA = static_cast<const float*>(p.A) + group_offset<0>(p.gL, l);
        const float* baseB = static_cast<const float*>(p.B) + group_offset<1>(p.gL, l);
        const BufRsrc A = Cfg::RAG ? make_rsrc(baseA, KOdometer::sgpr((uint32_t)(p.endA - (unsigned long long)(uintptr_t)baseA))) : make_rsrc(baseA);
        const BufRsrc B = Cfg::RAG ? make_rsrc(baseB, KOdometer::sgpr((uint32_t)(p.endB - (unsigned long long)(uintptr_t)baseB))) : make_rsrc(baseB);
        if constexpr (Cfg::ABL == 4) __builtin_amdgcn_s_setprio(3);
        OpA oa;
        OpB ob;
        oa.template init<0>(p.gM, p.gK, m0, wave, lane);
        ob.template init<1>(p.gN, p.gK, n0, wave, lane);
        KOdometer odo;
        odo.template init<Cfg::RAG>(p.gK, kBegin);
        const uint32_t kTilesAll = (p.gK.total + (uint32_t)BK - 1u) / (uint32_t)BK;
        const int maskAt = (Cfg::RAG && kBegin / (uint32_t)BK + (uint32_t)nTiles == kTilesAll) ? nTiles - 1 : 0x7fffffff;
        const uint32_t kValid = KOdometer::sgpr((p.gK.total % (uint32_t)BK) != 0u ? p.gK.total % (uint32_t)BK : (uint32_t)BK);
        int issued = 0;
        auto issue = [&](int slot) {
            float* stage = lds + slot * STAGE;
            constexpr int AUX = (Cfg::ABL == 5) ? 2 : 0;
            if constexpr (Cfg::RAG) {
                if (issued == maskAt) { oa.mask(wave, lane, kValid); ob.mask(wave, lane, kValid); }
                ++issued;
            }
            oa.template issue<AUX>(A, odo.offA, stage, wave);
            ob.template issue<AUX>(B, odo.offB, stage + OpA::FLOATS, wave);
            odo.advance(p.gK);
        };
        auto fix_last = [&]() {
            if constexpr (Cfg::RAG) {
                if (maskAt != 0x7fffffff && (kValid & 3u) != 0u) {
                    float* stage = lds + (maskAt % S) * STAGE;
                    oa.fix(stage, wave, lane, kValid);
                    ob.fix(stage + OpA::FLOATS, wave, lane, kValid);
                    asm volatile("s_waitcnt lgkmcnt(0)" ::: "memory");
                }
            }
        };
        if (tlog != nullptr && tid == 256) tlog[7] = __builtin_readcyclecounter();
        issue(0);
        if (nTiles > 1) {
            issue(1);
            CTAMD_WAIT_VMCNT(LOADS);
        } else {
            CTAMD_WAIT_VMCNT(0);
            fix_last();
        }
        __builtin_amdgcn_s_barrier();
#pragma unroll
        for (int T = 2; T < S; ++T)
            if (T < nTiles) issue(T);
        int slot = 0, t = 0;
        unsigned long long waitV = 0, waitB = 0;
        for (; t + S < nTiles; ++t) {
            unsigned long long c0 = 0, c1 = 0, c2 = 0;
            if constexpr (Cfg::ABL == 3) c0 = __builtin_readcyclecounter();
            if constexpr (Cfg::ABL == 1) CTAMD_WAIT_VMCNT(0); else CTAMD_WAIT_VMCNT(LOADS * (S - 2));
            if constexpr (Cfg::ABL == 3) c1 = __builtin_readcyclecounter();
            __builtin_amdgcn_s_barrier();
            if constexpr (Cfg::ABL == 3) { c2 = __builtin_readcyclecounter(); waitV += c1 - c0; waitB += c2 - c1; }
            if constexpr (Cfg::ABL != 1) issue(slot);
            slot = (slot + 1 == S) ? 0 : slot + 1;
        }
        if constexpr (Cfg::ABL == 3) {
            if (tlog != nullptr && tid == 256) { tlog[9] = waitV; tlog[10] = waitB; }
        }
        for (; t + 1 < nTiles; ++t) {
            const int behind = nTiles - t - 2;
            if (behind <= 0) { CTAMD_WAIT_VMCNT(0); fix_last(); }
            else if (behind == 1) CTAMD_WAIT_VMCNT(LOADS);
            else if (behind == 2) CTAMD_WAIT_VMCNT(LOADS * 2);
            else if (behind == 3) CTAMD_WAIT_VMCNT((S > 4 ? LOADS * 3 : 0));
            else CTAMD_WAIT_VMCNT((S > 5 ? LOADS * 4 : 0));
            __builtin_amdgcn_s_barrier();
        }
        CTAMD_WAIT_VMCNT(0);
        return;
    }

    __builtin_amdgcn_s_setprio(2);
    const int wm = wave & 1, wn = wave >> 1;
    f32x4 acc[TM][TN];
#pragma unroll
    for (int i = 0; i < TM; ++i)
#pragma unroll
        for (int j = 0; j < TN; ++j) acc[i][j] = f32x4{0.f, 0.f, 0.f, 0.f};

    int baseA[TM], baseB[TN];
#pragma unroll
    for (int i = 0; i < TM; ++i) baseA[i] = OpA::frag_base(wm * (BM / 2) + 16 * i, lane);
#pragma unroll
    for (int j = 0; j < TN; ++j) baseB[j] = OpB::frag_base(wn * (BN / 2) + 16 * j, lane);

    f32x4 a0[TM], b0[TN], a1[TM], b1[TN];
    auto load0 = [&](const float* st) {
#pragma unroll
        for (int i = 0; i < TM; ++i) a0[i] = OpA::template fragment<0>(st, baseA[i]);
#pragma unroll
        for (int j = 0; j < TN; ++j) b0[j] = OpB::template fragment<0>(st + OpA::FLOATS, baseB[j]);
    };
    auto load1 = [&](const float* st) {
#pragma unroll
        for (int i = 0; i < TM; ++i) a1[i] = OpA::template fragment<1>(st, baseA[i]);
#pragma unroll
        for (int j = 0; j < TN; ++j) b1[j] = OpB::template fragment<1>(st + OpA::FLOATS, baseB[j]);
    };
#define CTAMD_MFMA_RANGE(FA, FB, FIRST, LAST)                                                          \
    _Pragma("unroll") for (int kk = 0; kk < 4; ++kk)                                                   \
    _Pragma("unroll") for (int i = 0; i < TM; ++i)                                                     \
    _Pragma("unroll") for (int j = 0; j < TN; ++j) {                                                   \
        const int idx = (kk * TM + i) * TN + j;                                                        \
        if (Cfg::ABL != 2 && idx >= (FIRST) && idx < (LAST))                                           \
            acc[i][j] = __builtin_amdgcn_mfma_f32_16x16x4f32(FA[i][kk], FB[j][kk], acc[i][j], 0, 0, 0); \
    }
    constexpr int NMFMA = 4 * TM * TN;
    constexpr int SPLIT = NMFMA / 3;
#define CTAMD_INTERLEAVE_DS(n)                                         \
    _Pragma("unroll") for (int z = 0; z < (n); ++z) {                  \
        __builtin_amdgcn_sched_group_barrier(0x008, 1, 0);             \
        __builtin_amdgcn_sched_group_barrier(0x100, 1, 0);             \
    }

    __builtin_amdgcn_s_barrier();
    __builtin_amdgcn_sched_barrier(0);
    load0(lds);
    stamp(1);
    unsigned long long waitC = 0;

#define CTAMD_TILE_BODY(U, LASTTILE) CTAMD_TILE_BODY_AT(lds + (U) * STAGE, lds + (((U) + 1) % S) * STAGE, LASTTILE)
#define CTAMD_TILE_BODY_AT(CUR, NXT, LASTTILE) CTAMD_TILE_BODY_AT2(CUR, NXT, LASTTILE, load0, load1)
#define CTAMD_TILE_BODY_AT2(CUR, NXT, LASTTILE, load0, load1)                                              \
    {                                                                                                      \
        const float* cur = (CUR);                                                                          \
        const float* nxt = (NXT);                                                                          \
        load1(cur);                                                                                        \
        CTAMD_MFMA_RANGE(a0, b0, 0, NMFMA)                                                                 \
        CTAMD_INTERLEAVE_DS(TM + 4 * TN)                                                                   \
        __builtin_amdgcn_sched_barrier(0);                                                                 \
        CTAMD_MFMA_RANGE(a1, b1, 0, SPLIT)                                                                 \
        __builtin_amdgcn_sched_barrier(0);                                                                 \
        if constexpr (!(LASTTILE)) {                                                                       \
            asm volatile("s_waitcnt lgkmcnt(0)" ::: "memory");  \
            unsigned long long cb0 = 0;                                                                    \
            if constexpr (Cfg::ABL == 3) cb0 = __builtin_readcyclecounter();                               \
            __builtin_amdgcn_s_barrier();                                                                  \
            if constexpr (Cfg::ABL == 3) waitC += __builtin_readcyclecounter() - cb0;                      \
            __builtin_amdgcn_sched_barrier(0);                                                             \
            load0(nxt);                                                                                    \
            CTAMD_MFMA_RANGE(a1, b1, SPLIT, NMFMA)                                                         \
            CTAMD_INTERLEAVE_DS(TM + 4 * TN)                                                               \
        } else {                                                                                           \
            CTAMD_MFMA_RANGE(a1, b1, SPLIT, NMFMA)                                                         \
        }                                                                                                  \
        __builtin_amdgcn_sched_barrier(0);                                                                 \
    }
#define CTAMD_BODY_MID(U) CTAMD_TILE_BODY(U, false)
#define CTAMD_FOR_SLOTS(M)                                                     \
    { M(0) M(1) M(2)                                                           \
      if constexpr (S > 3) { M(3) } if constexpr (S > 4) { M(4) }              \
      if constexpr (S > 5) { M(5) } }
    int t = 0;
    for (; t + S < nTiles; t += S) CTAMD_FOR_SLOTS(CTAMD_BODY_MID)
    stamp(2);
    const int r = nTiles - t;
#define CTAMD_BODY_END(U) CTAMD_TILE_BODY(U, (U) == S - 1)
    if (r == S) {
        CTAMD_FOR_SLOTS(CTAMD_BODY_END)
    } else {
        auto opaque = [](int v) { asm volatile("" : "+v"(v)); return v; };
        auto load0t = [&](const float* st) {
#pragma unroll
            for (int i = 0; i < TM; ++i) a0[i] = OpA::template fragment<0>(st, opaque(baseA[i]));
#pragma unroll
            for (int j = 0; j < TN; ++j) b0[j] = OpB::template fragment<0>(st + OpA::FLOATS, opaque(baseB[j]));
        };
        auto load1t = [&](const float* st) {
#pragma unroll
            for (int i = 0; i < TM; ++i) a1[i] = OpA::template fragment<1>(st, opaque(baseA[i]));
#pragma unroll
            for (int j = 0; j < TN; ++j) b1[j] = OpB::template fragment<1>(st + OpA::FLOATS, opaque(baseB[j]));
        };
        int u = 0;
#pragma unroll 1
        for (; u + 1 < r; ++u) CTAMD_TILE_BODY_AT2(lds + u * STAGE, lds + (u + 1) * STAGE, false, load0t, load1t)
        CTAMD_TILE_BODY_AT2(lds + u * STAGE, lds, true, load0t, load1t)
    }
    stamp(3);
    if constexpr (Cfg::ABL == 3) {
        if (tlog != nullptr && wave8 == 0 && lane_now() == 0) tlog[8] = waitC;
    }

    const int laneE = lane_now();
    const int tidE = wave8 * 64 + laneE;
    const uint32_t Mtot = p.gM.total, Ntot = p.gN.total;
    if (p.partial != nullptr) {
        const size_t tileIdx = (((size_t)slice * p.gL.total + l) * p.tilesN + nt) * p.tilesM + mt;
        f32x4* P = reinterpret_cast<f32x4*>(p.partial) + (tileIdx * 4 + wave) * (size_t)(TM * TN * 64);
        const BufRsrc rP = make_rsrc(reinterpret_cast<const float*>(P));
        if (__builtin_expect(p.partialPolicy != 0, 0)) {
#pragma unroll
            for (int i = 0; i < TM; ++i)
#pragma unroll
                for (int j = 0; j < TN; ++j) {
                    if (p.partialPolicy == 1) store_policy_16<0>(acc[i][j], rP, (uint32_t)(((i * TN + j) * 64 + laneE) * 16));
                    else store_policy_16<2>(acc[i][j], rP, (uint32_t)(((i * TN + j) * 64 + laneE) * 16));
                }
        } else {
#pragma unroll
        for (int i = 0; i < TM; ++i)
#pragma unroll
            for (int j = 0; j < TN; ++j) store_wt_16(acc[i][j], rP, (uint32_t)(((i * TN + j) * 64 + laneE) * 16));
        }
        stamp(4);
        if (p.sync == nullptr) {
            stamp(6);
            return;
        }
        asm volatile("s_waitcnt vmcnt(0)" ::: "memory");
        __builtin_amdgcn_s_barrier();
        uint32_t* cnt = p.sync;
        if (tidE == 0) {
            __hip_atomic_fetch_add(cnt, 1u, __ATOMIC_RELAXED, __HIP_MEMORY_SCOPE_AGENT);
            uint32_t spins = 0;
            while (__hip_atomic_load(cnt, __ATOMIC_RELAXED, __HIP_MEMORY_SCOPE_AGENT) < p.nBlocks && ++spins < (1u << 22))
                __builtin_amdgcn_s_sleep(2);
            __builtin_amdgcn_fence(__ATOMIC_ACQUIRE, "agent");
            if (__hip_atomic_fetch_add(cnt + 1, 1u, __ATOMIC_RELAXED, __HIP_MEMORY_SCOPE_AGENT) == p.nBlocks - 1) {
                __hip_atomic_store(cnt, 0u, __ATOMIC_RELAXED, __HIP_MEMORY_SCOPE_AGENT);
                __hip_atomic_store(cnt + 1, 0u, __ATOMIC_RELAXED, __HIP_MEMORY_SCOPE_AGENT);
            }
        }
        __builtin_amdgcn_s_barrier();
        stamp(11);
        const uint32_t quadsTotal = p.tilesM * p.tilesN * 4u * TM * TN * 64u;
        const uint32_t lines = quadsTotal / 8u;
        const int q = tidE & 7, g = tidE >> 3;
        f32x4* red = reinterpret_cast<f32x4*>(lds);
        for (uint32_t line = blockIdx.x; line < lines; line += p.nBlocks) {
            const uint32_t e = line * 8u + q;
            const f32x4* src = reinterpret_cast<const f32x4*>(p.partial) + e;
            f32x4 sum = {0.f, 0.f, 0.f, 0.f};
            for (uint32_t s0 = g; s0 < p.splitK; s0 += 256) {
                f32x4 x[8];
#pragma unroll
                for (int u = 0; u < 8; ++u) {
                    const uint32_t sl = s0 + 32u * u;
                    x[u] = (sl < p.splitK) ? __builtin_nontemporal_load(src + (size_t)sl * quadsTotal) : f32x4{0.f, 0.f, 0.f, 0.f};
                }
                sum += ((x[0] + x[1]) + (x[2] + x[3])) + ((x[4] + x[5]) + (x[6] + x[7]));
            }
#pragma unroll
            for (int m = 8; m < 64; m <<= 1)
#pragma unroll
                for (int c = 0; c < 4; ++c) sum[c] += __shfl_xor(sum[c], m, 64);
            if (laneE < 8) red[wave * 8 + q] = sum;
            __builtin_amdgcn_s_barrier();
            if (tidE < 8) {
                sum = (red[q] + red[8 + q]) + (red[16 + q] + red[24 + q]);
                uint32_t rem = e;
                const uint32_t ln = rem % 64; rem /= 64;
                const uint32_t fj = rem % TN; rem /= TN;
                const uint32_t fi = rem % TM; rem /= TM;
                const uint32_t w = rem % 4; rem /= 4;
                const uint32_t tmt = rem % p.tilesM;
                const uint32_t tnt = rem / p.tilesM;
                const uint32_t n = tnt * BN + (w >> 1) * (BN / 2) + 16 * fj + (ln & 15);
                if (n < Ntot) {
#pragma unroll
                    for (int r = 0; r < 4; ++r) {
                        const uint32_t m = tmt * BM + (w & 1) * (BM / 2) + 16 * fi + 4 * (ln >> 4) + r;
                        if (m >= Mtot) continue;
                        float val = p.alpha * sum[r];
                        if (p.beta != 0.f)
                            val += p.beta * static_cast<const float*>(p.C)[(int64_t)m * p.cStrideM[0] + (int64_t)n * p.cStrideN[0]];
                        static_cast<float*>(p.D)[(int64_t)m * p.gM.stride[1][0] + (int64_t)n * p.gN.stride[1][0]] = val;
                    }
                }
            }
            __builtin_amdgcn_s_barrier();
        }
        stamp(6);
        return;
    }
    {
        constexpr int IMG = gett_f32_image_floats<TN>();
        static_assert(4 * IMG <= STAGE, "four per-wave row images fit one ring slot");
        const GettArgPtr q = gett_arg_ptr();
        const float* Cl;
        float* Dl;
        if (gett_f32_rows_ok(q, l, Cl, Dl)) {
            gett_store_tile_f32_rows<TM, TN>(q, Cl, Dl, acc, m0 + wm * (BM / 2), n0 + wn * (BN / 2), laneE, lds + (size_t)(nTiles % S) * STAGE + wave * IMG);
            stamp(4);
            stamp(6);
            return;
        }
    }
    const float* C = static_cast<const float*>(p.C);
    float*       D = static_cast<float*>(p.D);
    {
        int64_t oD, oC;
        group_offset2<2>(p.gL, p.cStrideL, l, oD, oC);
        D += oD;
        C += oC;
    }
    int64_t offDn[TN], offCn[TN];
    bool    okN[TN];
#pragma unroll
    for (int j = 0; j < TN; ++j) {
        const uint32_t n = n0 + wn * (BN / 2) + 16 * j + (laneE & 15);
        okN[j] = n < Ntot;
        offDn[j] = 0;
        offCn[j] = 0;
        if (okN[j]) group_offset2<1>(p.gN, p.cStrideN, n, offDn[j], offCn[j]);
    }
    const float alpha = p.alpha, beta = p.beta;
    bool vecD = p.gM.stride[1][0] == 1 && (p.gM.div[0].d & 3u) == 0u && (reinterpret_cast<uintptr_t>(D) & 15u) == 0u;
    bool vecC = vecD && p.cStrideM[0] == 1 && (reinterpret_cast<uintptr_t>(C) & 15u) == 0u;
#pragma unroll
    for (int q = 0; q < kMaxGroupModes; ++q) {
        vecD = vecD && (q == 0 || (p.gM.stride[1][q] & 3) == 0) && (p.gN.stride[1][q] & 3) == 0;
        vecC = vecC && (q == 0 || (p.cStrideM[q] & 3) == 0) && (p.cStrideN[q] & 3) == 0;
    }
    if (vecD) {
#pragma unroll
        for (int i = 0; i < TM; ++i) {
            const uint32_t m = m0 + wm * (BM / 2) + 16 * i + 4 * (laneE >> 4);
            if (m >= Mtot) continue;
            int64_t offDm, offCm;
            group_offset2<1>(p.gM, p.cStrideM, m, offDm, offCm);
#pragma unroll
            for (int j = 0; j < TN; ++j) {
                if (!okN[j]) continue;
                f32x4 val = {alpha * acc[i][j][0], alpha * acc[i][j][1], alpha * acc[i][j][2], alpha * acc[i][j][3]};
                if (beta != 0.f) {
                    const float* c = C + offCm + offCn[j];
                    if (vecC) {
                        const f32x4 cv = *reinterpret_cast<const f32x4*>(c);
                        val[0] += beta * cv[0]; val[1] += beta * cv[1]; val[2] += beta * cv[2]; val[3] += beta * cv[3];
                    } else {
                        int64_t dD, dC1, dC2, dC3;
                        group_offset2<1>(p.gM, p.cStrideM, m + 1, dD, dC1);
                        group_offset2<1>(p.gM, p.cStrideM, m + 2, dD, dC2);
                        group_offset2<1>(p.gM, p.cStrideM, m + 3, dD, dC3);
                        val[0] += beta * c[0];
                        val[1] += beta * C[dC1 + offCn[j]];
                        val[2] += beta * C[dC2 + offCn[j]];
                        val[3] += beta * C[dC3 + offCn[j]];
                    }
                }
                __builtin_nontemporal_store(val, reinterpret_cast<f32x4*>(D + offDm + offDn[j]));
            }
        }
        stamp(4);
        stamp(6);
        return;
    }
#pragma unroll
    for (int i = 0; i < TM; ++i)
#pragma unroll
        for (int r = 0; r < 4; ++r) {
            const uint32_t m = m0 + wm * (BM / 2) + 16 * i + 4 * (laneE >> 4) + r;
            if (m >= Mtot) continue;
            int64_t offDm, offCm;
            group_offset2<1>(p.gM, p.cStrideM, m, offDm, offCm);
#pragma unroll
            for (int j = 0; j < TN; ++j) {
                if (!okN[j]) continue;
                float val = alpha * acc[i][j][r];
                if (beta != 0.f) val += beta * C[offCm + offCn[j]];
                D[offDm + offDn[j]] = val;
            }
        }
    stamp(4);
    stamp(6);
}

__global__ void __launch_bounds__(256) splitk_reduce_frag_kernel(const SplitKReduceParams p) {
    __shared__ f32x4 red[4][8];
    const int q = threadIdx.x & 7, g = threadIdx.x >> 3;
    const uint32_t quadsPerTile = 4u * p.fragTM * p.fragTN * 64u;
    const size_t   tilesTotal = (size_t)p.gL.total * p.tilesN * p.tilesM;
    const size_t   quadsTotal = tilesTotal * quadsPerTile;
    const size_t   e = (size_t)blockIdx.x * 8 + q;
    f32x4 sum = {0.f, 0.f, 0.f, 0.f};
    if (e < quadsTotal) {
        const f32x4* src = reinterpret_cast<const f32x4*>(p.partial) + e;
        for (uint32_t s0 = g; s0 < p.splitK; s0 += 256) {
            f32x4 x[8];
#pragma unroll
            for (int u = 0; u < 8; ++u) {
                const uint32_t sl = s0 + 32u * u;
                x[u] = (sl < p.splitK) ? __builtin_nontemporal_load(src + (size_t)sl * quadsTotal) : f32x4{0.f, 0.f, 0.f, 0.f};
            }
            sum += ((x[0] + x[1]) + (x[2] + x[3])) + ((x[4] + x[5]) + (x[6] + x[7]));
        }
    }
#pragma unroll
    for (int m = 8; m < 64; m <<= 1)
#pragma unroll
        for (int c = 0; c < 4; ++c) sum[c] += __shfl_xor(sum[c], m, 64);
    const int wave = threadIdx.x >> 6;
    if ((threadIdx.x & 63) < 8) red[wave][q] = sum;
    __syncthreads();
    if (threadIdx.x >= 8 || e >= quadsTotal) return;
    sum = (red[0][q] + red[1][q]) + (red[2][q] + red[3][q]);
    size_t rem = e;
    const uint32_t lane = (uint32_t)(rem % 64); rem /= 64;
    const uint32_t j = (uint32_t)(rem % p.fragTN); rem /= p.fragTN;
    const uint32_t i = (uint32_t)(rem % p.fragTM); rem /= p.fragTM;
    const uint32_t w = (uint32_t)(rem % 4); rem /= 4;
    const uint32_t mt = (uint32_t)(rem % p.tilesM); rem /= p.tilesM;
    const uint32_t nt = (uint32_t)(rem % p.tilesN); rem /= p.tilesN;
    const uint32_t l = (uint32_t)rem;
    const uint32_t bm = 32u * p.fragTM, bn = 32u * p.fragTN;
    const uint32_t n = nt * bn + (w >> 1) * (bn / 2) + 16 * j + (lane & 15);
    if (n >= p.gN.total) return;
    int64_t oDl = 0, oCl = 0, oDn, oCn;
    group_offset2<2>(p.gL, p.cStrideL, l, oDl, oCl);
    group_offset2<1>(p.gN, p.cStrideN, n, oDn, oCn);
#pragma unroll
    for (int r = 0; r < 4; ++r) {
        const uint32_t m = mt * bm + (w & 1) * (bm / 2) + 16 * i + 4 * (lane >> 4) + r;
        if (m >= p.gM.total) continue;
        int64_t oDm, oCm;
        group_offset2<1>(p.gM, p.cStrideM, m, oDm, oCm);
        float val = p.alpha * sum[r];
        if (p.beta != 0.f) val += p.beta * static_cast<const float*>(p.C)[oCl + oCm + oCn];
        static_cast<float*>(p.D)[oDl + oDm + oDn] = val;
    }
}

struct FoldFlatParams {
    const float* partial;
    const float* C;
    float*       D;
    int64_t      sDm, sDn, sCm, sCn;
    float        alpha, beta;
    uint32_t     splitK, quadsTotal, fragTM, fragTN, tilesM, Mtot, Ntot;
};

template <int NT>
__global__ void __launch_bounds__(NT) splitk_reduce_frag_flat_kernel(const FoldFlatParams p) {
    constexpr int G = NT / 8, U = 256 / G, W = NT / 64;
    __shared__ f32x4 red[W][8];
    const int q = threadIdx.x & 7, g = threadIdx.x >> 3;
    const uint32_t e = blockIdx.x * 8 + q;
    f32x4 sum = {0.f, 0.f, 0.f, 0.f};
    if (e < p.quadsTotal) {
        const f32x4* src = reinterpret_cast<const f32x4*>(p.partial) + e;
        for (uint32_t s0 = g; s0 < p.splitK; s0 += 256) {
            f32x4 x[U];
#pragma unroll
            for (int u = 0; u < U; ++u) {
                const uint32_t sl = s0 + (uint32_t)G * u;
                x[u] = (sl < p.splitK) ? __builtin_nontemporal_load(src + (size_t)sl * p.quadsTotal) : f32x4{0.f, 0.f, 0.f, 0.f};
            }
#pragma unroll
            for (int st = 1; st < U; st <<= 1)
#pragma unroll
                for (int u = 0; u + st < U; u += 2 * st) x[u] += x[u + st];
            sum += x[0];
        }
    }
#pragma unroll
    for (int m = 8; m < 64; m <<= 1)
#pragma unroll
        for (int c = 0; c < 4; ++c) sum[c] += __shfl_xor(sum[c], m, 64);
    const int wave = threadIdx.x >> 6;
    if ((threadIdx.x & 63) < 8) red[wave][q] = sum;
    __syncthreads();
    if (threadIdx.x >= 8 || e >= p.quadsTotal) return;
    sum = red[0][q];
#pragma unroll
    for (int w = 1; w < W; ++w) sum += red[w][q];
    uint32_t rem = e;
    const uint32_t lane = rem % 64; rem /= 64;
    const uint32_t j = rem % p.fragTN; rem /= p.fragTN;
    const uint32_t i = rem % p.fragTM; rem /= p.fragTM;
    const uint32_t w = rem % 4; rem /= 4;
    const uint32_t mt = rem % p.tilesM;
    const uint32_t nt = rem / p.tilesM;
    const uint32_t bm = 32u * p.fragTM, bn = 32u * p.fragTN;
    const uint32_t n = nt * bn + (w >> 1) * (bn / 2) + 16 * j + (lane & 15);
    if (n >= p.Ntot) return;
#pragma unroll
    for (int r = 0; r < 4; ++r) {
        const uint32_t m = mt * bm + (w & 1) * (bm / 2) + 16 * i + 4 * (lane >> 4) + r;
        if (m >= p.Mtot) continue;
        float val = p.alpha * sum[r];
        if (p.beta != 0.f) val += p.beta * p.C[(int64_t)m * p.sCm + (int64_t)n * p.sCn];
        p.D[(int64_t)m * p.sDm + (int64_t)n * p.sDn] = val;
    }
}

hipError_t launch_splitk_reduce_frag(const SplitKReduceParams& p, hipStream_t stream) {
    const size_t quads = (size_t)p.gL.total * p.tilesN * p.tilesM * 4u * p.fragTM * p.fragTN * 64u;
    const size_t blocks = (quads + 7) / 8;
    if (blocks == 0) return hipSuccess;
    if (p.gL.total == 1 && p.gM.n <= 1 && p.gN.n <= 1 && quads < (1ull << 31)) {
        FoldFlatParams f;
        f.partial = p.partial;
        f.C = static_cast<const float*>(p.C);
        f.D = static_cast<float*>(p.D);
        f.sDm = p.gM.stride[1][0]; f.sDn = p.gN.stride[1][0];
        f.sCm = p.cStrideM[0];     f.sCn = p.cStrideN[0];
        f.alpha = p.alpha; f.beta = p.beta;
        f.splitK = p.splitK; f.quadsTotal = (uint32_t)quads;
        f.fragTM = p.fragTM; f.fragTN = p.fragTN; f.tilesM = p.tilesM;
        f.Mtot = p.gM.total; f.Ntot = p.gN.total;
        hipLaunchKernelGGL(splitk_reduce_frag_flat_kernel<256>, dim3((unsigned)blocks), dim3(256), 0, stream, f);
        return hipGetLastError();
    }
    hipLaunchKernelGGL(splitk_reduce_frag_kernel, dim3((unsigned)blocks), dim3(256), 0, stream, p);
    return hipGetLastError();
}

template <class Cfg>
static hipError_t launch_stream(const GettParams& p, hipStream_t stream) {
    if constexpr (Cfg::ABL == 0) {
        if (p.gK.total % (uint32_t)kStreamBK != 0u || (p.ragged & 1u) != 0u) {
            using R = StreamCfg<Cfg::BM, Cfg::BN, Cfg::LA, Cfg::LB, 4, 0, true>;
            hipLaunchKernelGGL(gett_f32_stream_kernel<R>, dim3(p.nBlocks), dim3(512), 0, stream, p);
            return hipGetLastError();
        }
    }
    hipLaunchKernelGGL(gett_f32_stream_kernel<Cfg>, dim3(p.nBlocks), dim3(512), 0, stream, p);
    return hipGetLastError();
}

#define CTAMD_STREAM_KERNELS(XS)        \
    XS(96, 96, LAY_K, LAY_F, 4)         \
    XS(96, 96, LAY_K, LAY_F, 6)         \
    XS(96, 96, LAY_K, LAY_F, 3)         \
    XS(96, 96, LAY_F, LAY_F, 4)         \
    XS(96, 96, LAY_F, LAY_K, 4)         \
    XS(96, 96, LAY_K, LAY_K, 4)         \
    XS(128, 128, LAY_F, LAY_F, 4)       \
    XS(128, 128, LAY_K, LAY_F, 4)       \
    XS(128, 128, LAY_F, LAY_K, 4)       \
    XS(128, 128, LAY_K, LAY_K, 4)       \
    XS(64, 64, LAY_F, LAY_F, 4)         \
    XS(64, 64, LAY_K, LAY_F, 4)         \
    XS(64, 64, LAY_F, LAY_K, 4)         \
    XS(64, 64, LAY_K, LAY_K, 4)         \
    XS(96, 96, LAY_F, LAY_F, 3)         \
    XS(96, 96, LAY_F, LAY_K, 3)         \
    XS(96, 96, LAY_K, LAY_K, 3)         \
    XS(128, 128, LAY_F, LAY_F, 3)       \
    XS(128, 128, LAY_K, LAY_F, 3)

#define CTAMD_STREAM_ENTRY(bm, bn, la, lb, s) \
    {bm, bn, kStreamBK, 2, 2, 1, la, lb, 512, s, 1, 0, &launch_stream<StreamCfg<bm, bn, la, lb, s>>, 1, 0, 0, 0, "gett_f32_stream_kernel"},

#define CTAMD_STREAM_ABL(bm, bn, la, lb, s, abl) \
    {bm, bn, kStreamBK, 2, 2, 1, la, lb, 512, s, 1, abl, &launch_stream<StreamCfg<bm, bn, la, lb, s, abl>>, 1, 0, 0, 0, "gett_f32_stream_kernel"},

#define CTAMD_STREAM_NT(bm, bn, la, lb, s) \
    {bm, bn, kStreamBK, 2, 2, 1, la, lb, 512, s, 1, 0, &launch_stream<StreamCfg<bm, bn, la, lb, s, 5>>, 1, 1, 0, 0, "gett_f32_stream_kernel"},

static const GettKernelInfo g_stream_table[] = {
    CTAMD_STREAM_KERNELS(CTAMD_STREAM_ENTRY)
    CTAMD_STREAM_ABL(96, 96, LAY_K, LAY_F, 4, 1)
    CTAMD_STREAM_ABL(96, 96, LAY_K, LAY_F, 4, 2)
    CTAMD_STREAM_ABL(96, 96, LAY_K, LAY_F, 4, 3)
    CTAMD_STREAM_ABL(96, 96, LAY_K, LAY_F, 4, 4)
    CTAMD_STREAM_NT(96, 96, LAY_K, LAY_F, 3) CTAMD_STREAM_NT(96, 96, LAY_F, LAY_F, 3)
    CTAMD_STREAM_NT(96, 96, LAY_F, LAY_K, 3) CTAMD_STREAM_NT(96, 96, LAY_K, LAY_K, 3)};

const GettKernelInfo* gett_f32_stream_kernels(int* count) {
    *count = (int)(sizeof(g_stream_table) / sizeof(g_stream_table[0]));
    return g_stream_table;
}

}
```

### cudalibrarysamples_amd/csrc/kernels/launch.h

```cpp
#pragma once
#include <hip/hip_runtime_api.h>

#include "params.h"

namespace ctamd {

enum OperandLayout : int {
    LAY_F = 0,
    LAY_K = 1,
    LAY_S = 2
};

enum H16Variant : int {
    H16_W8 = 0, H16_W4 = 8, H16_S = 16, H16_W4S = 24, H16_W4R = 32, H16_W4V = 40,
    H16_W4X  = 48,
    H16_W4M  = 56,
    H16_W4M4 = 64,
    H16_W8M  = 72,
    H16_W4Q  = 80,
    H16_W4P  = 88
};
constexpr int h16_entry(H16Variant variant, int layoutIdx) { return (int)variant + layoutIdx; }

struct GettKernelInfo {
    int bm, bn, bk;
    int wm, wn, wk;
    int layA, layB;
    int threads;
    int pf;
    int kfast;
    int ablation;
    hipError_t (*launch)(const GettParams&, hipStream_t);
    int fragPartials;
    int nt;
    int elem;
    int vec;
    const char* name;
    int variant;
};

enum GenElem : int { GEN_BF16 = 0, GEN_F16 = 1, GEN_F64 = 2, GEN_C32 = 3, GEN_C64 = 4,
                     GEN_F32_BF16 = 5, GEN_F32_F16 = 6, GEN_F32_BF16X3 = 7,
                     GEN_F64_F32 = 8, GEN_C64_C32 = 9 };
inline bool gen_elem_is_f32x(int elem) { return elem >= GEN_F32_BF16 && elem <= GEN_F32_BF16X3; }
inline bool gen_elem_is_f64x(int elem) { return elem == GEN_F64_F32 || elem == GEN_C64_C32; }
inline bool gen_elem_f32_partials(int elem) { return elem == GEN_BF16 || elem == GEN_F16 || gen_elem_is_f32x(elem); }
inline unsigned gen_elem_partial_bytes(int elem) {
    return (gen_elem_f32_partials(elem) || elem == GEN_F64_F32) ? 4u : (elem == GEN_C64) ? 16u : 8u;
}

const GettKernelInfo* gett_f32_kernels(int* count);
hipError_t launch_splitk_reduce(const SplitKReduceParams& p, hipStream_t stream);
hipError_t launch_splitk_reduce_frag(const SplitKReduceParams& p, hipStream_t stream);
const GettKernelInfo* gett_f32_stream_kernels(int* count);

const GettKernelInfo* gett_h16_kernels(int* count);
const GettKernelInfo* gett_h16v_kernels(int* count);
const GettKernelInfo* gett_h16p_kernels(int* count);

const GettKernelInfo* gett_gen_kernels(int* count);
const GettKernelInfo* gett_gen_h16_kernels(int* count);
const GettKernelInfo* gett_gen_f64_kernels(int* count);
const GettKernelInfo* gett_gen_cplx_kernels(int* count);
const GettKernelInfo* gett_gen_f32x_kernels(int* count);
const GettKernelInfo* gett_gen_f64x_kernels(int* count);
hipError_t launch_gen_splitk_reduce(const SplitKReduceParams& p, int elem, hipStream_t stream);
hipError_t launch_gen_f64x_splitk_reduce(const SplitKReduceParams& p, int elem, hipStream_t stream);

hipError_t launch_gett_simple(const GettParams& p, int dtype , bool accumulate64,
                              hipStream_t stream);

hipError_t launch_gett_wide(const WideParams& p, int dtype , bool accumulate64, hipStream_t stream);

enum EwVariant : int {
    EW_TRANSPOSE = 0,
    EW_ROWCOPY   = 1,
    EW_GENERIC   = 2,
    EW_TRANSPOSE_ANY = 4,
    EW_BLOCK     = 3
};
hipError_t launch_elementwise(const Ew2DParams& p, int variant, int dtype, hipStream_t stream);
hipError_t launch_elementwise_convert(const Ew2DParams& p, int variant, int dtypeA, int dtypeD, hipStream_t stream);
hipError_t launch_fill(void* D, uint64_t n, int dtype, double value, hipStream_t stream);

enum ReduceVariant : int {
    RED_COL     = 0,
    RED_ROW     = 1,
    RED_GENERIC = 2
};
hipError_t launch_reduce(const ReduceParams& p, int variant, int dtype, bool acc64, hipStream_t stream);
hipError_t launch_reduce_finalize(const ReduceParams& p, int dtype, bool acc64, hipStream_t stream);

}
```

### cudalibrarysamples_amd/csrc/kernels/params.h

```cpp
#pragma once
#include <stdint.h>

namespace ctamd {

constexpr int kMaxGroupModes = 4;

struct FastDiv {
    uint32_t d;
    uint32_t magic;
    uint32_t shift;
};

struct ModeGroup {
    int32_t  n;
    uint32_t total;
    FastDiv  div[kMaxGroupModes];
    int64_t  stride[3][kMaxGroupModes];
};

struct GettParams {
    const void* A;
    const void* B;
    const void* C;
    void*       D;
    float*      partial;
    unsigned long long* timing;
    uint32_t*   sync;
    unsigned long long xcdTiles;
    ModeGroup   gM, gN, gK, gL;
    float       alpha, beta;
    double      alpha64, beta64;
    uint32_t    tilesM, tilesN;
    uint32_t    splitK;
    uint32_t    kPerSlice;
    uint32_t    nBlocks;
    int64_t     cStrideM[kMaxGroupModes];
    int64_t     cStrideN[kMaxGroupModes];
    int64_t     cStrideL[kMaxGroupModes];
    double      alphaIm, betaIm;
    int32_t     conjA, conjB, conjC;
    int32_t     partialPolicy;
    unsigned long long endA, endB;
    uint32_t    ragged;
    uint32_t    mOrg, nOrg;
    uint32_t    tilesM2, tilesN2, mOrg2, nOrg2;
};

struct WideMode {
    FastDiv div;
    int64_t sA, sB, sC, sD;
};
struct WideParams {
    const void* A;
    const void* B;
    const void* C;
    void*       D;
    const WideMode* modes;
    uint32_t    nOut, nK;
    uint64_t    outTotal;
    uint32_t    kTotal;
    float       alpha, beta;
    double      alpha64, beta64;
    double      alphaIm, betaIm;
    int32_t     conjA, conjB, conjC;
};

struct SplitKReduceParams {
    const float* partial;
    const void*  C;
    void*        D;
    ModeGroup    gM, gN, gL;
    int64_t      cStrideM[kMaxGroupModes];
    int64_t      cStrideN[kMaxGroupModes];
    int64_t      cStrideL[kMaxGroupModes];
    float        alpha, beta;
    uint32_t     splitK;
    uint32_t     tilesM, tilesN;
    uint32_t     fragTM, fragTN;
    int32_t      outType;
    double       alpha64, beta64, alphaIm, betaIm;
    int32_t      conjC;
};

struct Ew2DParams {
    const void* A;
    const void* C;
    void*       D;
    uint32_t    E0, E1;
    int64_t     sA0, sA1, sD0, sD1, sC0, sC1;
    uint32_t    tiles0, tiles1;
    uint32_t    tile0;
    uint32_t    tile1;
    uint32_t    order;
    uint32_t    idsPerXcd;
    FastDiv     divRest;
    FastDiv     divTiles0, divTiles1;
    ModeGroup   rest;
    uint32_t    nBlocks;
    float       alpha, gamma;
    double      alpha64, gamma64;
    const void* E;
    float       delta;
    double      delta64;
    int32_t     opAB, opAC;
    const void* X;
    int64_t     sX0, sX1;
    int64_t     restX[kMaxGroupModes];
    float       xi;
    uint8_t     unA, unX, unE, unC;
    double      xi64;
    double      alphaIm, gammaIm;
    int32_t     conjA, conjC;
    uint32_t    blkN, blkTotal, blkGroup, blkBlocks;
    uint32_t    blkVec;
    FastDiv     blkDiv[4];
    uint32_t    blkSrc[4];
    ModeGroup   blkRest;
};

struct ReduceParams {
    const void* A;
    const void* C;
    void*       D;
    void*       partial;
    ModeGroup   kept;
    ModeGroup   red;
    uint32_t    splitR;
    uint32_t    redPerSplit;
    int32_t     op;
    float       alpha, beta;
    double      alpha64, beta64;
    double      alphaIm, betaIm;
    int32_t     conjA, conjC;
    uint32_t    rowAny;
    uint8_t     unA, unC;
};

}
```

### cudalibrarysamples_amd/cutensor.py

```python
import ctypes
import os

_HERE = os.path.dirname(os.path.abspath(__file__))
LIB_DIR = "lib_hooks" if os.environ.get("CTAMD_LIB_FLAVOUR") == "hooks" else "lib"
LIB_PATH = os.environ.get("CUTENSOR_AMD_LIBRARY") or os.path.join(_HERE, LIB_DIR, "libcutensor.so")

if not os.path.exists(LIB_PATH):
    raise ImportError(
        "libcutensor.so (gfx950 HIP engine) is not built: %s missing. Build it with "
        "`make -C cudalibrarysamples_amd/csrc` or `__graft_entry__.build()`; there is no CPU fallback." % LIB_PATH)

lib = ctypes.CDLL(LIB_PATH, mode=ctypes.RTLD_GLOBAL)
if LIB_DIR == "lib" and not os.environ.get("CUTENSOR_AMD_LIBRARY"):
    _ignored = sorted(k for k in os.environ if k.startswith(("CUTENSOR_AMD_", "CUTENSORMP_AMD_")) and k != "CUTENSOR_AMD_LIBRARY")
    if _ignored:
        import warnings
        warnings.warn("the production libcutensor.so does not read %s: set CTAMD_LIB_FLAVOUR=hooks to load the test-hooks flavour" % ", ".join(_ignored))

R_32F, R_64F, R_16F, R_16BF = 0, 1, 2, 14
C_32F, C_64F = 4, 5
STATUS_SUCCESS, STATUS_NOT_INITIALIZED, STATUS_INVALID_VALUE = 0, 1, 7
STATUS_NOT_SUPPORTED, STATUS_INSUFFICIENT_WORKSPACE, STATUS_IO_ERROR = 15, 19, 21
OP_IDENTITY, OP_ADD, OP_MUL, OP_MAX, OP_MIN = 1, 3, 5, 6, 7
OP_CONJ = 9
OP_SQRT, OP_RELU, OP_RCP, OP_SIGMOID, OP_TANH, OP_EXP, OP_LOG, OP_ABS, OP_NEG = 2, 8, 10, 11, 12, 22, 23, 24, 25
ALGO_DEFAULT, ALGO_DEFAULT_PATIENT = -1, -6
WORKSPACE_MIN, WORKSPACE_DEFAULT, WORKSPACE_MAX = 1, 2, 3
JIT_MODE_NONE = 0
OPERATION_DESCRIPTOR_TAG, OPERATION_DESCRIPTOR_SCALAR_TYPE, OPERATION_DESCRIPTOR_FLOPS, OPERATION_DESCRIPTOR_MOVED_BYTES = 0, 1, 2, 3
PLAN_REQUIRED_WORKSPACE = 0
PLAN_PREFERENCE_AUTOTUNE_MODE, PLAN_PREFERENCE_CACHE_MODE, PLAN_PREFERENCE_INCREMENTAL_COUNT = 0, 1, 2
PLAN_PREFERENCE_ALGO, PLAN_PREFERENCE_KERNEL_RANK = 3, 4
AMD_PLAN_PREFERENCE_OPERANDS_STREAMED = 1000
AUTOTUNE_MODE_NONE, AUTOTUNE_MODE_INCREMENTAL = 0, 1
CACHE_MODE_NONE, CACHE_MODE_PEDANTIC = 0, 1

_vp = ctypes.c_void_p
_i64p = ctypes.POINTER(ctypes.c_int64)
_i32p = ctypes.POINTER(ctypes.c_int32)

EXPORTS = {
    "cutensorCreate": (ctypes.POINTER(_vp),),
    "cutensorDestroy": (_vp,),
    "cutensorHandleResizePlanCache": (_vp, ctypes.c_uint32),
    "cutensorHandleWritePlanCacheToFile": (_vp, ctypes.c_char_p),
    "cutensorHandleReadPlanCacheFromFile": (_vp, ctypes.c_char_p, ctypes.POINTER(ctypes.c_uint32)),
    "cutensorCreateTensorDescriptor": (_vp, ctypes.POINTER(_vp), ctypes.c_uint32, _i64p, _i64p, ctypes.c_int, ctypes.c_uint32),
    "cutensorDestroyTensorDescriptor": (_vp,),
    "cutensorCreateContraction": (_vp, ctypes.POINTER(_vp), _vp, _i32p, ctypes.c_int, _vp, _i32p, ctypes.c_int,
                                  _vp, _i32p, ctypes.c_int, _vp, _i32p, _vp),
    "cutensorCreateReduction": (_vp, ctypes.POINTER(_vp), _vp, _i32p, ctypes.c_int, _vp, _i32p, ctypes.c_int,
                                _vp, _i32p, ctypes.c_int, _vp),
    "cutensorCreatePermutation": (_vp, ctypes.POINTER(_vp), _vp, _i32p, ctypes.c_int, _vp, _i32p, _vp),
    "cutensorCreateElementwiseBinary": (_vp, ctypes.POINTER(_vp), _vp, _i32p, ctypes.c_int, _vp, _i32p, ctypes.c_int,
                                        _vp, _i32p, ctypes.c_int, _vp),
    "cutensorDestroyOperationDescriptor": (_vp,),
    "cutensorOperationDescriptorGetAttribute": (_vp, _vp, ctypes.c_int, _vp, ctypes.c_size_t),
    "cutensorOperationDescriptorSetAttribute": (_vp, _vp, ctypes.c_int, _vp, ctypes.c_size_t),
    "cutensorCreatePlanPreference": (_vp, ctypes.POINTER(_vp), ctypes.c_int, ctypes.c_int),
    "cutensorDestroyPlanPreference": (_vp,),
    "cutensorPlanPreferenceSetAttribute": (_vp, _vp, ctypes.c_int, _vp, ctypes.c_size_t),
    "cutensorEstimateWorkspaceSize": (_vp, _vp, _vp, ctypes.c_int, ctypes.POINTER(ctypes.c_uint64)),
    "cutensorCreatePlan": (_vp, ctypes.POINTER(_vp), _vp, _vp, ctypes.c_uint64),
    "cutensorDestroyPlan": (_vp,),
    "cutensorPlanGetAttribute": (_vp, _vp, ctypes.c_int, _vp, ctypes.c_size_t),
    "cutensorContract": (_vp, _vp, _vp, _vp, _vp, _vp, _vp, _vp, _vp, ctypes.c_uint64, _vp),
    "cutensorReduce": (_vp, _vp, _vp, _vp, _vp, _vp, _vp, _vp, ctypes.c_uint64, _vp),
    "cutensorPermute": (_vp, _vp, _vp, _vp, _vp, _vp),
    "cutensorElementwiseBinaryExecute": (_vp, _vp, _vp, _vp, _vp, _vp, _vp, _vp),
    "cutensorCreateElementwiseTrinary": (_vp, ctypes.POINTER(_vp), _vp, _i32p, ctypes.c_int, _vp, _i32p, ctypes.c_int,
                                         _vp, _i32p, ctypes.c_int, _vp, _i32p, ctypes.c_int, ctypes.c_int, _vp),
    "cutensorElementwiseTrinaryExecute": (_vp, _vp, _vp, _vp, _vp, _vp, _vp, _vp, _vp, _vp),
    "cutensorCreateContractionTrinary": (_vp, ctypes.POINTER(_vp), _vp, _i32p, ctypes.c_int, _vp, _i32p, ctypes.c_int,
                                         _vp, _i32p, ctypes.c_int, _vp, _i32p, ctypes.c_int, _vp, _i32p, _vp),
    "cutensorContractTrinary": (_vp, _vp, _vp, _vp, _vp, _vp, _vp, _vp, _vp, _vp, ctypes.c_uint64, _vp),
    "cutensorCreateBlockSparseTensorDescriptor": (_vp, ctypes.POINTER(_vp), ctypes.c_uint32, ctypes.c_uint64, ctypes.POINTER(ctypes.c_uint32),
                                                  _i64p, _i32p, _i64p, ctypes.c_int),
    "cutensorDestroyBlockSparseTensorDescriptor": (_vp,),
    "cutensorCreateBlockSparseContraction": (_vp, ctypes.POINTER(_vp), _vp, _i32p, ctypes.c_int, _vp, _i32p, ctypes.c_int,
                                             _vp, _i32p, ctypes.c_int, _vp, _i32p, _vp),
    "cutensorBlockSparseContract": (_vp, _vp, _vp, ctypes.POINTER(_vp), ctypes.POINTER(_vp), _vp, ctypes.POINTER(_vp), ctypes.POINTER(_vp),
                                    _vp, ctypes.c_uint64, _vp),
    "cutensorReadKernelCacheFromFile": (_vp, ctypes.c_char_p),
    "cutensorWriteKernelCacheToFile": (_vp, ctypes.c_char_p),
}
DATA_SYMBOLS = ["CUTENSOR_COMPUTE_DESC_16F", "CUTENSOR_COMPUTE_DESC_16BF", "CUTENSOR_COMPUTE_DESC_TF32",
                "CUTENSOR_COMPUTE_DESC_3XTF32", "CUTENSOR_COMPUTE_DESC_32F", "CUTENSOR_COMPUTE_DESC_64F"]

for _name, _args in EXPORTS.items():
    _f = getattr(lib, _name)
    _f.argtypes = list(_args)
    _f.restype = ctypes.c_int
    globals()[_name] = _f
lib.cutensorGetErrorString.argtypes = [ctypes.c_int]
lib.cutensorGetErrorString.restype = ctypes.c_char_p
lib.cutensorGetVersion.restype = ctypes.c_size_t
lib.ctamdDescribePlan.argtypes = [_vp, ctypes.c_char_p, ctypes.c_size_t]
lib.ctamdCountCandidates.argtypes = [_vp, _vp, ctypes.c_uint64]
lib.ctamdPlanMemoStats.argtypes = [_vp, ctypes.POINTER(ctypes.c_uint64), ctypes.POINTER(ctypes.c_uint64), ctypes.POINTER(ctypes.c_uint32)]
lib.ctamdPlanMemoStats.restype = None
lib.ctamdLaunchCounts.argtypes = [ctypes.POINTER(ctypes.c_uint64)]
lib.ctamdLaunchCounts.restype = None
lib.ctamdLastH16Kernel.argtypes = []
lib.ctamdLastH16Kernel.restype = ctypes.c_int
lib.ctamdSetTimingBuffer.argtypes = [_vp, _vp]
lib.ctamdSetTimingBuffer.restype = None
lib.ctamdSetSplitKFold.argtypes = [_vp, ctypes.c_int]
lib.ctamdSetSplitKFold.restype = None
lib.ctamdProfileBegin.argtypes = [_vp]
lib.ctamdProfileBegin.restype = None
lib.ctamdProfileEnd.argtypes = [_vp, ctypes.POINTER(ctypes.c_float), ctypes.POINTER(ctypes.c_float)]
lib.ctamdEinsumCreate.argtypes = [ctypes.c_char_p, _i64p, ctypes.c_int, _i64p, ctypes.c_int, ctypes.c_int]
lib.ctamdEinsumCreate.restype = _vp
lib.ctamdEinsumSetConjugate.argtypes = [_vp, ctypes.c_int, ctypes.c_int]
lib.ctamdEinsumSetConjugate.restype = None
lib.ctamdEinsumSetCompute.argtypes = [_vp, ctypes.c_int]
lib.ctamdEinsumSetCompute.restype = None
lib.ctamdEinsumDestroy.argtypes = [_vp]
lib.ctamdEinsumDestroy.restype = None
lib.ctamdEinsumIsInitialized.argtypes = [_vp]
lib.ctamdEinsumOutputShape.argtypes = [_vp, _i64p, ctypes.c_int]
lib.ctamdEinsumPlan.argtypes = [_vp, _vp, ctypes.c_uint64, ctypes.POINTER(ctypes.c_uint64)]
lib.ctamdEinsumReplan.argtypes = [_vp, _vp, ctypes.c_uint64, ctypes.POINTER(ctypes.c_uint64)]
lib.ctamdEinsumReplan.restype = ctypes.c_int
lib.ctamdMeasureMfmaCeiling.argtypes = [ctypes.c_int, ctypes.c_int, ctypes.POINTER(ctypes.c_float)]
lib.ctamdMeasureMfmaCeiling.restype = ctypes.c_int
lib.ctamdMeasureMfmaCeilingShape.argtypes = [ctypes.c_int, ctypes.c_int, ctypes.c_int, ctypes.POINTER(ctypes.c_float)]
lib.ctamdMeasureMfmaCeilingShape.restype = ctypes.c_int
lib.ctamdEinsumExecute.argtypes = [_vp, _vp, _vp, _vp, _vp, _vp, _vp]
lib.ctamdEinsumRawPlan.argtypes = [_vp]
lib.ctamdEinsumRawPlan.restype = _vp


def plan_memo_stats(handle):
    h, m, e = ctypes.c_uint64(0), ctypes.c_uint64(0), ctypes.c_uint32(0)
    lib.ctamdPlanMemoStats(handle, ctypes.byref(h), ctypes.byref(m), ctypes.byref(e))
    return h.value, m.value, e.value


def launch_counts():
    out = (ctypes.c_uint64 * 5)()
    lib.ctamdLaunchCounts(out)
    return dict(zip(("simple", "wide", "f32", "h16", "gen"), [int(v) for v in out]))


def last_h16_kernel():
    return int(lib.ctamdLastH16Kernel())


def compute_desc(name):
    return _vp.in_dll(lib, "CUTENSOR_COMPUTE_DESC_" + name)


class CuTensorError(RuntimeError):
    def __init__(self, status):
        self.status = status
        RuntimeError.__init__(self, lib.cutensorGetErrorString(status).decode())


def check(status):
    if status != STATUS_SUCCESS:
        raise CuTensorError(status)


def getErrorString(status):
    return lib.cutensorGetErrorString(status).decode()


def describe_plan(plan):
    buf = ctypes.create_string_buffer(1024)
    lib.ctamdDescribePlan(plan, buf, 1024)
    import json
    return json.loads(buf.value.decode())


def i64(values):
    return (ctypes.c_int64 * max(len(values), 1))(*values)


def i32(values):
    return (ctypes.c_int32 * max(len(values), 1))(*[ord(v) if isinstance(v, str) else int(v) for v in values])
```

Baseline: 114,700.

## Add flat-start f32 stream kernel entry with compact 128-byte parameters

Adds a second entry point for the f32 streaming GETT kernel that takes a compact 128-byte parameter block and walks the flattened contracted modes with magic-number division and incremental offset stepping. The goal is to cut kernel-argument and setup overhead at block start. The existing ring and k-loop bodies move into shared include files so both entries can use them. Env hooks are added to disable the flat start and to force the split-K factor, plus a counter of flat-start launches. The extra path adds complexity and could pick a different kernel variant at runtime.

Result: faster. 118,800 (median of 6 runs) (+3.5%).

```diff
diff --git a/cudalibrarysamples_amd/csrc/host/api.cpp b/cudalibrarysamples_amd/csrc/host/api.cpp
--- a/cudalibrarysamples_amd/csrc/host/api.cpp
+++ b/cudalibrarysamples_amd/csrc/host/api.cpp
@@ -145,7 +145,7 @@
            CTAMD_HOOK_ENV("CUTENSOR_AMD_H16_TRANSPOSE_T1") || CTAMD_HOOK_ENV("CUTENSOR_AMD_NT") || CTAMD_HOOK_ENV("CUTENSOR_AMD_H16_WAVES") || CTAMD_HOOK_ENV("CUTENSOR_AMD_H16_SPLITK") ||
            CTAMD_HOOK_ENV("CUTENSOR_AMD_KORDER") || CTAMD_HOOK_ENV("CUTENSOR_AMD_ABLATION") || CTAMD_HOOK_ENV("CUTENSOR_AMD_PEEL") || CTAMD_HOOK_ENV("CUTENSOR_AMD_GEN") ||
            CTAMD_HOOK_ENV("CUTENSOR_AMD_REPACK") || CTAMD_HOOK_ENV("CUTENSOR_AMD_EW_ANY") || CTAMD_HOOK_ENV("CUTENSOR_AMD_F32X") ||
-           CTAMD_HOOK_ENV("CUTENSOR_AMD_F64X");
+           CTAMD_HOOK_ENV("CUTENSOR_AMD_F64X") || CTAMD_HOOK_ENV("CUTENSOR_AMD_F32_SPLITK");
 }
 
 double scalar_as_double(const void* s, hipDataType t) {
@@ -1838,6 +1838,7 @@
     if (c.family == 0) {
         static const int policy = [] { const char* e = CTAMD_HOOK_ENV("CUTENSOR_AMD_PARTIAL_STORE"); return e ? (e[0] == 'p' ? 1 : e[0] == 'n' ? 2 : e[0] == 's' ? 3 : 0) : 0; }();
         p.partialPolicy = policy;
+        p.noFlatStart = CTAMD_HOOK_ENV_IS("CUTENSOR_AMD_FLAT_START", '0') ? 1 : 0;
         if (plan.fusedFold) {
             uint32_t slot;
             {
@@ -1861,6 +1862,7 @@
     r.partial = static_cast<float*>(workspace);
     r.C = p.C; r.D = p.D; r.alpha = p.alpha; r.beta = p.beta;
     r.alpha64 = s.a; r.beta64 = s.b; r.alphaIm = s.aIm; r.betaIm = s.bIm; r.conjC = p.conjC;
+    r.noFlatStart = p.noFlatStart;
     return launch_splitk_fold(c.family, tab[c.kernel], r, stream);
 }
 
@@ -2142,6 +2144,8 @@
 void ctamdLaunchCounts(uint64_t out[5]) try {
     for (int i = 0; i < 5; ++i) out[i] = g_launchCounts[i].load(std::memory_order_relaxed);
 } CTAMD_API_CATCH_VOID
+
+uint64_t ctamdFlatStartCount(void) try { return g_flatStartLaunches.load(std::memory_order_relaxed); } CTAMD_API_CATCH_ZERO
 
 void ctamdPlanMemoStats(const cutensorHandle_t handle, uint64_t* hits, uint64_t* misses, uint32_t* entries) try {
     if (handle == nullptr) return;
diff --git a/cudalibrarysamples_amd/csrc/host/plan_contraction.cpp b/cudalibrarysamples_amd/csrc/host/plan_contraction.cpp
--- a/cudalibrarysamples_amd/csrc/host/plan_contraction.cpp
+++ b/cudalibrarysamples_amd/csrc/host/plan_contraction.cpp
@@ -343,6 +343,10 @@
             if (tiles * s > (uint64_t)numCUs * 16) break;
             splits.push_back(s);
         }
+        if (const char* fs = CTAMD_HOOK_ENV("CUTENSOR_AMD_F32_SPLITK")) {
+            const uint64_t want = std::strtoull(fs, nullptr, 10);
+            if (want >= 2 && want <= kTiles) splits = {(uint32_t)want};
+        }
         for (uint32_t s : splits) {
             ContractionChoice c;
             c.kernel = i;
diff --git a/cudalibrarysamples_amd/csrc/kernels/gett_f32_stream.hip b/cudalibrarysamples_amd/csrc/kernels/gett_f32_stream.hip
--- a/cudalibrarysamples_amd/csrc/kernels/gett_f32_stream.hip
+++ b/cudalibrarysamples_amd/csrc/kernels/gett_f32_stream.hip
@@ -1,6 +1,8 @@
 #include <hip/hip_runtime.h>
 #include <stdint.h>
 #include <stdlib.h>
+
+#include <atomic>
 
 #include "params.h"
 #include "launch.h"
@@ -80,6 +82,27 @@
         }
     }
 
+    __device__ __forceinline__ void init_flat(uint32_t strideBytes, uint32_t total, uint32_t strideK0Bytes, int wave, int lane) {
+#pragma unroll
+        for (int i = 0; i < PER_WAVE; ++i) {
+            const int c = wave + 4 * i;
+            if constexpr (LAY == LAY_K) {
+                const int r = 8 * c + (lane >> 3), p = lane & 7;
+                const int u = p ^ ((r >> 1) & 7);
+                uint32_t row = (uint32_t)r;
+                if (row >= total) row = total - 1;
+                src[i] = row * strideBytes + 16u * (uint32_t)u;
+            } else {
+                const int g = 64 * c + lane;
+                const int kr = g / UR, p = g % UR;
+                const int u = (p + 4 * ((kr >> 2) & 1)) % UR;
+                uint32_t row = 4u * (uint32_t)u;
+                if (row >= total) row = (total - 1u) & ~3u;
+                src[i] = row * strideBytes + (uint32_t)kr * strideK0Bytes;
+            }
+        }
+    }
+
     template <int AUX = 0>
     __device__ __forceinline__ void issue(BufRsrc X, uint32_t offKBytes, float* stage, int wave) const {
 #pragma unroll
@@ -182,6 +205,48 @@
             }
         }
     }
+    __device__ static __forceinline__ uint32_t flat_div(const StreamFlatParams& f, int i, uint32_t n) {
+        return __umulhi(n, f.kMagic[i]) >> ((f.kShifts >> (8 * i)) & 0xffu);
+    }
+    __device__ static __forceinline__ void flat_high(const StreamFlatParams& f, uint32_t hi, uint32_t& a, uint32_t& b) {
+        const uint32_t d3 = flat_div(f, 2, hi), d2 = hi - d3 * f.kExt[2];
+        a = d2 * f.kStrideA[2] + d3 * f.kStrideA[3];
+        b = d2 * f.kStrideB[2] + d3 * f.kStrideB[3];
+    }
+    __device__ __forceinline__ void init(const StreamFlatParams& f, uint32_t k0) {
+        const uint32_t E0 = f.kExt[0];
+        n0 = sgpr(E0 / kStreamBK);
+        e1 = sgpr(f.kExt[1]);
+        const uint32_t q0 = flat_div(f, 0, k0), d0 = k0 - q0 * E0;
+        j0 = sgpr(d0 / kStreamBK);
+        hi = sgpr((e1 < 2) ? q0 : flat_div(f, 1, q0));
+        j1 = sgpr(q0 - hi * e1);
+        uint32_t a, b;
+        flat_high(f, hi, a, b);
+        offA = sgpr(d0 * f.kStrideA[0] + j1 * f.kStrideA[1] + a);
+        offB = sgpr(d0 * f.kStrideB[0] + j1 * f.kStrideB[1] + b);
+        stepA = sgpr((uint32_t)kStreamBK * f.kStrideA[0]);
+        stepB = sgpr((uint32_t)kStreamBK * f.kStrideB[0]);
+        wrapA = sgpr(f.kStrideA[1] - (n0 - 1) * stepA);
+        wrapB = sgpr(f.kStrideB[1] - (n0 - 1) * stepB);
+    }
+    __device__ __forceinline__ void advance(const StreamFlatParams& f) {
+        const bool c0 = (j0 + 1 == n0);
+        j0 = c0 ? 0u : j0 + 1;
+        offA += c0 ? wrapA : stepA;
+        offB += c0 ? wrapB : stepB;
+        j1 += c0 ? 1u : 0u;
+        if (j1 == e1) {
+            j1 = 0;
+            hi += 1;
+            if (hi * e1 * f.kExt[0] < f.kTotal) {
+                uint32_t a, b;
+                flat_high(f, hi, a, b);
+                offA = sgpr(a);
+                offB = sgpr(b);
+            }
+        }
+    }
 };
 
 template <int BM_, int BN_, int LA_, int LB_, int S_, int ABL_ = 0, bool RAG_ = false>
@@ -189,6 +254,8 @@
     static constexpr int BM = BM_, BN = BN_, LA = LA_, LB = LB_, S = S_;
     static constexpr bool RAG = RAG_;
     static constexpr int ABL = ABL_;
+    static constexpr bool FLAT = ABL_ == 6 || ABL_ == 7;
+    static constexpr bool NT = ABL_ == 5 || ABL_ == 7;
     static constexpr int TM = BM / 32, TN = BN / 32;
 };
 
@@ -270,7 +337,7 @@
         int issued = 0;
         auto issue = [&](int slot) {
             float* stage = lds + slot * STAGE;
-            constexpr int AUX = (Cfg::ABL == 5) ? 2 : 0;
+            constexpr int AUX = Cfg::NT ? 2 : 0;
             if constexpr (Cfg::RAG) {
                 if (issued == maskAt) { oa.mask(wave, lane, kValid); ob.mask(wave, lane, kValid); }
                 ++issued;
@@ -289,158 +356,10 @@
                 }
             }
         };
-        if (tlog != nullptr && tid == 256) tlog[7] = __builtin_readcyclecounter();
-        issue(0);
-        if (nTiles > 1) {
-            issue(1);
-            CTAMD_WAIT_VMCNT(LOADS);
-        } else {
-            CTAMD_WAIT_VMCNT(0);
-            fix_last();
-        }
-        __builtin_amdgcn_s_barrier();
-#pragma unroll
-        for (int T = 2; T < S; ++T)
-            if (T < nTiles) issue(T);
-        int slot = 0, t = 0;
-        unsigned long long waitV = 0, waitB = 0;
-        for (; t + S < nTiles; ++t) {
-            unsigned long long c0 = 0, c1 = 0, c2 = 0;
-            if constexpr (Cfg::ABL == 3) c0 = __builtin_readcyclecounter();
-            if constexpr (Cfg::ABL == 1) CTAMD_WAIT_VMCNT(0); else CTAMD_WAIT_VMCNT(LOADS * (S - 2));
-            if constexpr (Cfg::ABL == 3) c1 = __builtin_readcyclecounter();
-            __builtin_amdgcn_s_barrier();
-            if constexpr (Cfg::ABL == 3) { c2 = __builtin_readcyclecounter(); waitV += c1 - c0; waitB += c2 - c1; }
-            if constexpr (Cfg::ABL != 1) issue(slot);
-            slot = (slot + 1 == S) ? 0 : slot + 1;
-        }
-        if constexpr (Cfg::ABL == 3) {
-            if (tlog != nullptr && tid == 256) { tlog[9] = waitV; tlog[10] = waitB; }
-        }
-        for (; t + 1 < nTiles; ++t) {
-            const int behind = nTiles - t - 2;
-            if (behind <= 0) { CTAMD_WAIT_VMCNT(0); fix_last(); }
-            else if (behind == 1) CTAMD_WAIT_VMCNT(LOADS);
-            else if (behind == 2) CTAMD_WAIT_VMCNT(LOADS * 2);
-            else if (behind == 3) CTAMD_WAIT_VMCNT((S > 4 ? LOADS * 3 : 0));
-            else CTAMD_WAIT_VMCNT((S > 5 ? LOADS * 4 : 0));
-            __builtin_amdgcn_s_barrier();
-        }
-        CTAMD_WAIT_VMCNT(0);
-        return;
-    }
-
-    __builtin_amdgcn_s_setprio(2);
-    const int wm = wave & 1, wn = wave >> 1;
-    f32x4 acc[TM][TN];
-#pragma unroll
-    for (int i = 0; i < TM; ++i)
-#pragma unroll
-        for (int j = 0; j < TN; ++j) acc[i][j] = f32x4{0.f, 0.f, 0.f, 0.f};
-
-    int baseA[TM], baseB[TN];
-#pragma unroll
-    for (int i = 0; i < TM; ++i) baseA[i] = OpA::frag_base(wm * (BM / 2) + 16 * i, lane);
-#pragma unroll
-    for (int j = 0; j < TN; ++j) baseB[j] = OpB::frag_base(wn * (BN / 2) + 16 * j, lane);
-
-    f32x4 a0[TM], b0[TN], a1[TM], b1[TN];
-    auto load0 = [&](const float* st) {
-#pragma unroll
-        for (int i = 0; i < TM; ++i) a0[i] = OpA::template fragment<0>(st, baseA[i]);
-#pragma unroll
-        for (int j = 0; j < TN; ++j) b0[j] = OpB::template fragment<0>(st + OpA::FLOATS, baseB[j]);
-    };
-    auto load1 = [&](const float* st) {
-#pragma unroll
-        for (int i = 0; i < TM; ++i) a1[i] = OpA::template fragment<1>(st, baseA[i]);
-#pragma unroll
-        for (int j = 0; j < TN; ++j) b1[j] = OpB::template fragment<1>(st + OpA::FLOATS, baseB[j]);
-    };
-#define CTAMD_MFMA_RANGE(FA, FB, FIRST, LAST)                                                          \
-    _Pragma("unroll") for (int kk = 0; kk < 4; ++kk)                                                   \
-    _Pragma("unroll") for (int i = 0; i < TM; ++i)                                                     \
-    _Pragma("unroll") for (int j = 0; j < TN; ++j) {                                                   \
-        const int idx = (kk * TM + i) * TN + j;                                                        \
-        if (Cfg::ABL != 2 && idx >= (FIRST) && idx < (LAST))                                           \
-            acc[i][j] = __builtin_amdgcn_mfma_f32_16x16x4f32(FA[i][kk], FB[j][kk], acc[i][j], 0, 0, 0); \
-    }
-    constexpr int NMFMA = 4 * TM * TN;
-    constexpr int SPLIT = NMFMA / 3;
-#define CTAMD_INTERLEAVE_DS(n)                                         \
-    _Pragma("unroll") for (int z = 0; z < (n); ++z) {                  \
-        __builtin_amdgcn_sched_group_barrier(0x008, 1, 0);             \
-        __builtin_amdgcn_sched_group_barrier(0x100, 1, 0);             \
-    }
-
-    __builtin_amdgcn_s_barrier();
-    __builtin_amdgcn_sched_barrier(0);
-    load0(lds);
-    stamp(1);
-    unsigned long long waitC = 0;
-
-#define CTAMD_TILE_BODY(U, LASTTILE) CTAMD_TILE_BODY_AT(lds + (U) * STAGE, lds + (((U) + 1) % S) * STAGE, LASTTILE)
-#define CTAMD_TILE_BODY_AT(CUR, NXT, LASTTILE) CTAMD_TILE_BODY_AT2(CUR, NXT, LASTTILE, load0, load1)
-#define CTAMD_TILE_BODY_AT2(CUR, NXT, LASTTILE, load0, load1)                                              \
-    {                                                                                                      \
-        const float* cur = (CUR);                                                                          \
-        const float* nxt = (NXT);                                                                          \
-        load1(cur);                                                                                        \
-        CTAMD_MFMA_RANGE(a0, b0, 0, NMFMA)                                                                 \
-        CTAMD_INTERLEAVE_DS(TM + 4 * TN)                                                                   \
-        __builtin_amdgcn_sched_barrier(0);                                                                 \
-        CTAMD_MFMA_RANGE(a1, b1, 0, SPLIT)                                                                 \
-        __builtin_amdgcn_sched_barrier(0);                                                                 \
-        if constexpr (!(LASTTILE)) {                                                                       \
-            asm volatile("s_waitcnt lgkmcnt(0)" ::: "memory");  \
-            unsigned long long cb0 = 0;                                                                    \
-            if constexpr (Cfg::ABL == 3) cb0 = __builtin_readcyclecounter();                               \
-            __builtin_amdgcn_s_barrier();                                                                  \
-            if constexpr (Cfg::ABL == 3) waitC += __builtin_readcyclecounter() - cb0;                      \
-            __builtin_amdgcn_sched_barrier(0);                                                             \
-            load0(nxt);                                                                                    \
-            CTAMD_MFMA_RANGE(a1, b1, SPLIT, NMFMA)                                                         \
-            CTAMD_INTERLEAVE_DS(TM + 4 * TN)                                                               \
-        } else {                                                                                           \
-            CTAMD_MFMA_RANGE(a1, b1, SPLIT, NMFMA)                                                         \
-        }                                                                                                  \
-        __builtin_amdgcn_sched_barrier(0);                                                                 \
-    }
-#define CTAMD_BODY_MID(U) CTAMD_TILE_BODY(U, false)
-#define CTAMD_FOR_SLOTS(M)                                                     \
-    { M(0) M(1) M(2)                                                           \
-      if constexpr (S > 3) { M(3) } if constexpr (S > 4) { M(4) }              \
-      if constexpr (S > 5) { M(5) } }
-    int t = 0;
-    for (; t + S < nTiles; t += S) CTAMD_FOR_SLOTS(CTAMD_BODY_MID)
-    stamp(2);
-    const int r = nTiles - t;
-#define CTAMD_BODY_END(U) CTAMD_TILE_BODY(U, (U) == S - 1)
-    if (r == S) {
-        CTAMD_FOR_SLOTS(CTAMD_BODY_END)
-    } else {
-        auto opaque = [](int v) { asm volatile("" : "+v"(v)); return v; };
-        auto load0t = [&](const float* st) {
-#pragma unroll
-            for (int i = 0; i < TM; ++i) a0[i] = OpA::template fragment<0>(st, opaque(baseA[i]));
-#pragma unroll
-            for (int j = 0; j < TN; ++j) b0[j] = OpB::template fragment<0>(st + OpA::FLOATS, opaque(baseB[j]));
-        };
-        auto load1t = [&](const float* st) {
-#pragma unroll
-            for (int i = 0; i < TM; ++i) a1[i] = OpA::template fragment<1>(st, opaque(baseA[i]));
-#pragma unroll
-            for (int j = 0; j < TN; ++j) b1[j] = OpB::template fragment<1>(st + OpA::FLOATS, opaque(baseB[j]));
-        };
-        int u = 0;
-#pragma unroll 1
-        for (; u + 1 < r; ++u) CTAMD_TILE_BODY_AT2(lds + u * STAGE, lds + (u + 1) * STAGE, false, load0t, load1t)
-        CTAMD_TILE_BODY_AT2(lds + u * STAGE, lds, true, load0t, load1t)
-    }
-    stamp(3);
-    if constexpr (Cfg::ABL == 3) {
-        if (tlog != nullptr && wave8 == 0 && lane_now() == 0) tlog[8] = waitC;
-    }
+#include "gett_f32_stream_ring.inc"
+    }
+
+#include "gett_f32_stream_kloop.inc"
 
     const int laneE = lane_now();
     const int tidE = wave8 * 64 + laneE;
@@ -627,6 +546,77 @@
     stamp(6);
 }
 
+template <class Cfg>
+__global__ void __launch_bounds__(512, 2) gett_f32_stream_kernel(const StreamFlatParams p) {
+    static_assert(Cfg::FLAT && !Cfg::RAG, "the flat entry has no ragged form");
+    constexpr int BM = Cfg::BM, BN = Cfg::BN, BK = kStreamBK, S = Cfg::S;
+    constexpr int TM = Cfg::TM, TN = Cfg::TN;
+    using OpA = StreamOperand<Cfg::LA, BM>;
+    using OpB = StreamOperand<Cfg::LB, BN>;
+    constexpr int STAGE = OpA::FLOATS + OpB::FLOATS;
+    constexpr int LOADS = OpA::PER_WAVE + OpB::PER_WAVE;
+    static_assert(S >= 3 && S <= 6 && S * STAGE * 4 <= 160 * 1024, "LDS ring must fit 160 KiB");
+    static_assert(LOADS * (S - 1) <= 63, "vmcnt is a 6-bit counter");
+    __shared__ __attribute__((aligned(16))) float lds[S * STAGE];
+
+    const int tid  = threadIdx.x;
+    const int lane = tid & 63;
+    const int wave8 = __builtin_amdgcn_readfirstlane(tid >> 6);
+    const int wave = wave8 & 3;
+    const bool loader = wave8 >= 4;
+    unsigned long long* tlog = p.timing ? p.timing + (size_t)blockIdx.x * 16 : nullptr;
+    auto lane_now = []() -> int {
+#if defined(__HIP_DEVICE_COMPILE__)
+        return (int)__builtin_amdgcn_mbcnt_hi(~0u, __builtin_amdgcn_mbcnt_lo(~0u, 0u));
+#else
+        return 0;
+#endif
+    };
+    auto stamp = [&](int slot) {
+        if (tlog != nullptr && wave8 == 0 && lane_now() == 0) tlog[slot] = (slot >= 5 && slot != 7) ? wall_clock64() : __builtin_readcyclecounter();
+    };
+    stamp(0);
+    stamp(5);
+
+    const uint32_t slice = xcd_remap(blockIdx.x, p.nBlocks);
+    const uint32_t kBegin = slice * p.kPerSlice;
+    uint32_t kEnd = kBegin + p.kPerSlice;
+    if (kEnd > p.kTotal) kEnd = p.kTotal;
+    const int nTiles = (int)((kEnd - kBegin) / BK);
+
+    if (loader) {
+        const BufRsrc A = make_rsrc(p.A);
+        const BufRsrc B = make_rsrc(p.B);
+        OpA oa;
+        OpB ob;
+        oa.init_flat(p.sM, p.Mtot, p.kStrideA[0], wave, lane);
+        ob.init_flat(p.sN, p.Ntot, p.kStrideB[0], wave, lane);
+        KOdometer odo;
+        odo.init(p, kBegin);
+        auto issue = [&](int slot) {
+            float* stage = lds + slot * STAGE;
+            constexpr int AUX = Cfg::NT ? 2 : 0;
+            oa.template issue<AUX>(A, odo.offA, stage, wave);
+            ob.template issue<AUX>(B, odo.offB, stage + OpA::FLOATS, wave);
+            odo.advance(p);
+        };
+        auto fix_last = [] {};
+#include "gett_f32_stream_ring.inc"
+    }
+
+#include "gett_f32_stream_kloop.inc"
+
+    const int laneE = lane_now();
+    f32x4* P = reinterpret_cast<f32x4*>(p.partial) + ((size_t)slice * 4 + wave) * (size_t)(TM * TN * 64);
+    const BufRsrc rP = make_rsrc(reinterpret_cast<const float*>(P));
+#pragma unroll
+    for (int i = 0; i < TM; ++i)
+#pragma unroll
+        for (int j = 0; j < TN; ++j) store_wt_16(acc[i][j], rP, (uint32_t)(((i * TN + j) * 64 + laneE) * 16));
+    stamp(4);
+    stamp(6);
+}
+
 __global__ void __launch_bounds__(256) splitk_reduce_frag_kernel(const SplitKReduceParams p) {
     __shared__ f32x4 red[4][8];
     const int q = threadIdx.x & 7, g = threadIdx.x >> 3;
@@ -684,64 +674,82 @@
 
 struct FoldFlatParams {
     const float* partial;
+    uint32_t     splitK, quadsTotal;
+    float*       D;
     const float* C;
-    float*       D;
     int64_t      sDm, sDn, sCm, sCn;
     float        alpha, beta;
-    uint32_t     splitK, quadsTotal, fragTM, fragTN, tilesM, Mtot, Ntot;
+    uint32_t     tilesM, Mtot, Ntot;
+    uint32_t     fragTM, fragTN;
 };
 
-template <int NT>
+template <int NT, int FTM, int FTN>
 __global__ void __launch_bounds__(NT) splitk_reduce_frag_flat_kernel(const FoldFlatParams p) {
     constexpr int G = NT / 8, U = 256 / G, W = NT / 64;
     __shared__ f32x4 red[W][8];
     const int q = threadIdx.x & 7, g = threadIdx.x >> 3;
     const uint32_t e = blockIdx.x * 8 + q;
+    const bool live = e < p.quadsTotal;
+    const f32x4* src = reinterpret_cast<const f32x4*>(p.partial) + e;
+    auto load = [&](f32x4 (&x)[U], uint32_t s0) {
+#pragma unroll
+        for (int u = 0; u < U; ++u) {
+            const uint32_t sl = s0 + (uint32_t)G * u;
+            x[u] = (live && sl < p.splitK) ? __builtin_nontemporal_load(src + (size_t)sl * p.quadsTotal) : f32x4{0.f, 0.f, 0.f, 0.f};
+        }
+    };
+    auto tree = [](f32x4 (&x)[U]) {
+#pragma unroll
+        for (int st = 1; st < U; st <<= 1)
+#pragma unroll
+            for (int u = 0; u + st < U; u += 2 * st) x[u] += x[u + st];
+    };
+    f32x4 x[U];
+    load(x, (uint32_t)g);
+    const uint32_t fragTM = FTM ? (uint32_t)FTM : p.fragTM, fragTN = FTN ? (uint32_t)FTN : p.fragTN;
+    uint32_t rem = e;
+    const uint32_t lane = rem % 64; rem /= 64;
+    const uint32_t j = rem % fragTN; rem /= fragTN;
+    const uint32_t i = rem % fragTM; rem /= fragTM;
+    const uint32_t w = rem % 4; rem /= 4;
+    const uint32_t mt = (p.tilesM == 1u) ? 0u : rem % p.tilesM;
+    const uint32_t nt = (p.tilesM == 1u) ? rem : rem / p.tilesM;
+    const uint32_t bm = 32u * fragTM, bn = 32u * fragTN;
+    const uint32_t n = nt * bn + (w >> 1) * (bn / 2) + 16 * j + (lane & 15);
+    const uint32_t m0 = mt * bm + (w & 1) * (bm / 2) + 16 * i + 4 * (lane >> 4);
+    float* d = p.D + (int64_t)m0 * p.sDm + (int64_t)n * p.sDn;
+    const float* c = p.C + (int64_t)m0 * p.sCm + (int64_t)n * p.sCn;
+    tree(x);
     f32x4 sum = {0.f, 0.f, 0.f, 0.f};
-    if (e < p.quadsTotal) {
-        const f32x4* src = reinterpret_cast<const f32x4*>(p.partial) + e;
-        for (uint32_t s0 = g; s0 < p.splitK; s0 += 256) {
-            f32x4 x[U];
-#pragma unroll
-            for (int u = 0; u < U; ++u) {
-                const uint32_t sl = s0 + (uint32_t)G * u;
-                x[u] = (sl < p.splitK) ? __builtin_nontemporal_load(src + (size_t)sl * p.quadsTotal) : f32x4{0.f, 0.f, 0.f, 0.f};
-            }
-#pragma unroll
-            for (int st = 1; st < U; st <<= 1)
-#pragma unroll
-                for (int u = 0; u + st < U; u += 2 * st) x[u] += x[u + st];
-            sum += x[0];
-        }
+    sum += x[0];
+    for (uint32_t s0 = g + 256u; s0 < p.splitK; s0 += 256) {
+        load(x, s0);
+        tree(x);
+        sum += x[0];
     }
 #pragma unroll
     for (int m = 8; m < 64; m <<= 1)
 #pragma unroll
-        for (int c = 0; c < 4; ++c) sum[c] += __shfl_xor(sum[c], m, 64);
+        for (int cc = 0; cc < 4; ++cc) sum[cc] += __shfl_xor(sum[cc], m, 64);
     const int wave = threadIdx.x >> 6;
     if ((threadIdx.x & 63) < 8) red[wave][q] = sum;
     __syncthreads();
-    if (threadIdx.x >= 8 || e >= p.quadsTotal) return;
+    if (threadIdx.x >= 8 || !live || n >= p.Ntot) return;
     sum = red[0][q];
 #pragma unroll
-    for (int w = 1; w < W; ++w) sum += red[w][q];
-    uint32_t rem = e;
-    const uint32_t lane = rem % 64; rem /= 64;
-    const uint32_t j = rem % p.fragTN; rem /= p.fragTN;
-    const uint32_t i = rem % p.fragTM; rem /= p.fragTM;
-    const uint32_t w = rem % 4; rem /= 4;
-    const uint32_t mt = rem % p.tilesM;
-    const uint32_t nt = rem / p.tilesM;
-    const uint32_t bm = 32u * p.fragTM, bn = 32u * p.fragTN;
-    const uint32_t n = nt * bn + (w >> 1) * (bn / 2) + 16 * j + (lane & 15);
-    if (n >= p.Ntot) return;
+    for (int ww = 1; ww < W; ++ww) sum += red[ww][q];
+    if (p.beta == 0.f) {
+#pragma unroll
+        for (int r = 0; r < 4; ++r)
+            if (m0 + r < p.Mtot) d[r * p.sDm] = p.alpha * sum[r];
+        return;
+    }
 #pragma unroll
     for (int r = 0; r < 4; ++r) {
-        const uint32_t m = mt * bm + (w & 1) * (bm / 2) + 16 * i + 4 * (lane >> 4) + r;
-        if (m >= p.Mtot) continue;
+        if (m0 + r >= p.Mtot) continue;
         float val = p.alpha * sum[r];
-        if (p.beta != 0.f) val += p.beta * p.C[(int64_t)m * p.sCm + (int64_t)n * p.sCn];
-        p.D[(int64_t)m * p.sDm + (int64_t)n * p.sDn] = val;
+        val += p.beta * c[r * p.sCm];
+        d[r * p.sDm] = val;
     }
 }
 
@@ -760,11 +768,43 @@
         f.splitK = p.splitK; f.quadsTotal = (uint32_t)quads;
         f.fragTM = p.fragTM; f.fragTN = p.fragTN; f.tilesM = p.tilesM;
         f.Mtot = p.gM.total; f.Ntot = p.gN.total;
-        hipLaunchKernelGGL(splitk_reduce_frag_flat_kernel<256>, dim3((unsigned)blocks), dim3(256), 0, stream, f);
+        const dim3 grid((unsigned)blocks), block(256);
+        const uint32_t frag = (p.noFlatStart == 0 && p.fragTM == p.fragTN) ? p.fragTM : 0u;
+        if (frag == 2u) hipLaunchKernelGGL((splitk_reduce_frag_flat_kernel<256, 2, 2>), grid, block, 0, stream, f);
+        else if (frag == 3u) hipLaunchKernelGGL((splitk_reduce_frag_flat_kernel<256, 3, 3>), grid, block, 0, stream, f);
+        else if (frag == 4u) hipLaunchKernelGGL((splitk_reduce_frag_flat_kernel<256, 4, 4>), grid, block, 0, stream, f);
+        else hipLaunchKernelGGL((splitk_reduce_frag_flat_kernel<256, 0, 0>), grid, block, 0, stream, f);
         return hipGetLastError();
     }
     hipLaunchKernelGGL(splitk_reduce_frag_kernel, dim3((unsigned)blocks), dim3(256), 0, stream, p);
     return hipGetLastError();
+}
+
+std::atomic<uint64_t> g_flatStartLaunches{0};
+
+static bool flat_start_params(const GettParams& p, StreamFlatParams& f) {
+    if (p.noFlatStart != 0 || p.partial == nullptr || p.sync != nullptr || p.xcdTiles != 0 || p.partialPolicy != 0) return false;
+    if (p.gL.total != 1 || p.gM.n > 1 || p.gN.n > 1 || p.tilesM * p.tilesN != 1 || p.nBlocks != p.splitK) return false;
+    if (p.gK.total % (uint32_t)kStreamBK != 0u || p.gK.div[0].d % (uint32_t)kStreamBK != 0u || (p.ragged & 1u) != 0u) return false;
+    f.A = static_cast<const float*>(p.A);
+    f.B = static_cast<const float*>(p.B);
+    f.partial = p.partial;
+    f.timing = p.timing;
+    f.sM = (uint32_t)p.gM.stride[0][0] * 4u; f.sN = (uint32_t)p.gN.stride[0][0] * 4u;
+    f.Mtot = p.gM.total; f.Ntot = p.gN.total;
+    f.splitK = p.splitK; f.kPerSlice = p.kPerSlice; f.nBlocks = p.nBlocks;
+    f.kTotal = p.gK.total;
+    f.kShifts = 0;
+    for (int i = 0; i < kMaxGroupModes; ++i) {
+        f.kExt[i] = p.gK.div[i].d;
+        f.kStrideA[i] = (uint32_t)p.gK.stride[0][i] * 4u;
+        f.kStrideB[i] = (uint32_t)p.gK.stride[1][i] * 4u;
+        if (i < kMaxGroupModes - 1) {
+            f.kMagic[i] = p.gK.div[i].magic;
+            f.kShifts |= (p.gK.div[i].shift & 0xffu) << (8 * i);
+        }
+    }
+    return true;
 }
 
 template <class Cfg>
@@ -773,6 +813,15 @@
         if (p.gK.total % (uint32_t)kStreamBK != 0u || (p.ragged & 1u) != 0u) {
             using R = StreamCfg<Cfg::BM, Cfg::BN, Cfg::LA, Cfg::LB, 4, 0, true>;
             hipLaunchKernelGGL(gett_f32_stream_kernel<R>, dim3(p.nBlocks), dim3(512), 0, stream, p);
+            return hipGetLastError();
+        }
+    }
+    if constexpr (Cfg::BM == 96 && Cfg::BN == 96 && Cfg::S == 3 && (Cfg::ABL == 0 || Cfg::ABL == 5)) {
+        StreamFlatParams f;
+        if (flat_start_params(p, f)) {
+            using F = StreamCfg<96, 96, Cfg::LA, Cfg::LB, 3, Cfg::ABL == 0 ? 6 : 7>;
+            hipLaunchKernelGGL(gett_f32_stream_kernel<F>, dim3(p.nBlocks), dim3(512), 0, stream, f);
+            g_flatStartLaunches.fetch_add(1, std::memory_order_relaxed);
             return hipGetLastError();
         }
     }
diff --git a/cudalibrarysamples_amd/csrc/kernels/gett_f32_stream_kloop.inc b/cudalibrarysamples_amd/csrc/kernels/gett_f32_stream_kloop.inc
--- /dev/null
+++ b/cudalibrarysamples_amd/csrc/kernels/gett_f32_stream_kloop.inc
@@ -0,0 +1,111 @@
+    __builtin_amdgcn_s_setprio(2);
+    const int wm = wave & 1, wn = wave >> 1;
+    f32x4 acc[TM][TN];
+#pragma unroll
+    for (int i = 0; i < TM; ++i)
+#pragma unroll
+        for (int j = 0; j < TN; ++j) acc[i][j] = f32x4{0.f, 0.f, 0.f, 0.f};
+
+    int baseA[TM], baseB[TN];
+#pragma unroll
+    for (int i = 0; i < TM; ++i) baseA[i] = OpA::frag_base(wm * (BM / 2) + 16 * i, lane);
+#pragma unroll
+    for (int j = 0; j < TN; ++j) baseB[j] = OpB::frag_base(wn * (BN / 2) + 16 * j, lane);
+
+    f32x4 a0[TM], b0[TN], a1[TM], b1[TN];
+    auto load0 = [&](const float* st) {
+#pragma unroll
+        for (int i = 0; i < TM; ++i) a0[i] = OpA::template fragment<0>(st, baseA[i]);
+#pragma unroll
+        for (int j = 0; j < TN; ++j) b0[j] = OpB::template fragment<0>(st + OpA::FLOATS, baseB[j]);
+    };
+    auto load1 = [&](const float* st) {
+#pragma unroll
+        for (int i = 0; i < TM; ++i) a1[i] = OpA::template fragment<1>(st, baseA[i]);
+#pragma unroll
+        for (int j = 0; j < TN; ++j) b1[j] = OpB::template fragment<1>(st + OpA::FLOATS, baseB[j]);
+    };
+#define CTAMD_MFMA_RANGE(FA, FB, FIRST, LAST)                                                          \
+    _Pragma("unroll") for (int kk = 0; kk < 4; ++kk)                                                   \
+    _Pragma("unroll") for (int i = 0; i < TM; ++i)                                                     \
+    _Pragma("unroll") for (int j = 0; j < TN; ++j) {                                                   \
+        const int idx = (kk * TM + i) * TN + j;                                                        \
+        if (Cfg::ABL != 2 && idx >= (FIRST) && idx < (LAST))                                           \
+            acc[i][j] = __builtin_amdgcn_mfma_f32_16x16x4f32(FA[i][kk], FB[j][kk], acc[i][j], 0, 0, 0); \
+    }
+    constexpr int NMFMA = 4 * TM * TN;
+    constexpr int SPLIT = NMFMA / 3;
+#define CTAMD_INTERLEAVE_DS(n)                                         \
+    _Pragma("unroll") for (int z = 0; z < (n); ++z) {                  \
+        __builtin_amdgcn_sched_group_barrier(0x008, 1, 0);             \
+        __builtin_amdgcn_sched_group_barrier(0x100, 1, 0);             \
+    }
+
+    __builtin_amdgcn_s_barrier();
+    __builtin_amdgcn_sched_barrier(0);
+    load0(lds);
+    stamp(1);
+    unsigned long long waitC = 0;
+
+#define CTAMD_TILE_BODY(U, LASTTILE) CTAMD_TILE_BODY_AT(lds + (U) * STAGE, lds + (((U) + 1) % S) * STAGE, LASTTILE)
+#define CTAMD_TILE_BODY_AT(CUR, NXT, LASTTILE) CTAMD_TILE_BODY_AT2(CUR, NXT, LASTTILE, load0, load1)
+#define CTAMD_TILE_BODY_AT2(CUR, NXT, LASTTILE, load0, load1)                                              \
+    {                                                                                                      \
+        const float* cur = (CUR);                                                                          \
+        const float* nxt = (NXT);                                                                          \
+        load1(cur);                                                                                        \
+        CTAMD_MFMA_RANGE(a0, b0, 0, NMFMA)                                                                 \
+        CTAMD_INTERLEAVE_DS(TM + 4 * TN)                                                                   \
+        __builtin_amdgcn_sched_barrier(0);                                                                 \
+        CTAMD_MFMA_RANGE(a1, b1, 0, SPLIT)                                                                 \
+        __builtin_amdgcn_sched_barrier(0);                                                                 \
+        if constexpr (!(LASTTILE)) {                                                                       \
+            asm volatile("s_waitcnt lgkmcnt(0)" ::: "memory");  \
+            unsigned long long cb0 = 0;                                                                    \
+            if constexpr (Cfg::ABL == 3) cb0 = __builtin_readcyclecounter();                               \
+            __builtin_amdgcn_s_barrier();                                                                  \
+            if constexpr (Cfg::ABL == 3) waitC += __builtin_readcyclecounter() - cb0;                      \
+            __builtin_amdgcn_sched_barrier(0);                                                             \
+            load0(nxt);                                                                                    \
+            CTAMD_MFMA_RANGE(a1, b1, SPLIT, NMFMA)                                                         \
+            CTAMD_INTERLEAVE_DS(TM + 4 * TN)                                                               \
+        } else {                                                                                           \
+            CTAMD_MFMA_RANGE(a1, b1, SPLIT, NMFMA)                                                         \
+        }                                                                                                  \
+        __builtin_amdgcn_sched_barrier(0);                                                                 \
+    }
+#define CTAMD_BODY_MID(U) CTAMD_TILE_BODY(U, false)
+#define CTAMD_FOR_SLOTS(M)                                                     \
+    { M(0) M(1) M(2)                                                           \
+      if constexpr (S > 3) { M(3) } if constexpr (S > 4) { M(4) }              \
+      if constexpr (S > 5) { M(5) } }
+    int t = 0;
+    for (; t + S < nTiles; t += S) CTAMD_FOR_SLOTS(CTAMD_BODY_MID)
+    stamp(2);
+    const int r = nTiles - t;
+#define CTAMD_BODY_END(U) CTAMD_TILE_BODY(U, (U) == S - 1)
+    if (r == S) {
+        CTAMD_FOR_SLOTS(CTAMD_BODY_END)
+    } else {
+        auto opaque = [](int v) { asm volatile("" : "+v"(v)); return v; };
+        auto load0t = [&](const float* st) {
+#pragma unroll
+            for (int i = 0; i < TM; ++i) a0[i] = OpA::template fragment<0>(st, opaque(baseA[i]));
+#pragma unroll
+            for (int j = 0; j < TN; ++j) b0[j] = OpB::template fragment<0>(st + OpA::FLOATS, opaque(baseB[j]));
+        };
+        auto load1t = [&](const float* st) {
+#pragma unroll
+            for (int i = 0; i < TM; ++i) a1[i] = OpA::template fragment<1>(st, opaque(baseA[i]));
+#pragma unroll
+            for (int j = 0; j < TN; ++j) b1[j] = OpB::template fragment<1>(st + OpA::FLOATS, opaque(baseB[j]));
+        };
+        int u = 0;
+#pragma unroll 1
+        for (; u + 1 < r; ++u) CTAMD_TILE_BODY_AT2(lds + u * STAGE, lds + (u + 1) * STAGE, false, load0t, load1t)
+        CTAMD_TILE_BODY_AT2(lds + u * STAGE, lds, true, load0t, load1t)
+    }
+    stamp(3);
+    if constexpr (Cfg::ABL == 3) {
+        if (tlog != nullptr && wave8 == 0 && lane_now() == 0) tlog[8] = waitC;
+    }
diff --git a/cudalibrarysamples_amd/csrc/kernels/gett_f32_stream_ring.inc b/cudalibrarysamples_amd/csrc/kernels/gett_f32_stream_ring.inc
--- /dev/null
+++ b/cudalibrarysamples_amd/csrc/kernels/gett_f32_stream_ring.inc
@@ -0,0 +1,39 @@
+        if (tlog != nullptr && tid == 256) tlog[7] = __builtin_readcyclecounter();
+        issue(0);
+        if (nTiles > 1) {
+            issue(1);
+            CTAMD_WAIT_VMCNT(LOADS);
+        } else {
+            CTAMD_WAIT_VMCNT(0);
+            fix_last();
+        }
+        __builtin_amdgcn_s_barrier();
+#pragma unroll
+        for (int T = 2; T < S; ++T)
+            if (T < nTiles) issue(T);
+        int slot = 0, t = 0;
+        unsigned long long waitV = 0, waitB = 0;
+        for (; t + S < nTiles; ++t) {
+            unsigned long long c0 = 0, c1 = 0, c2 = 0;
+            if constexpr (Cfg::ABL == 3) c0 = __builtin_readcyclecounter();
+            if constexpr (Cfg::ABL == 1) CTAMD_WAIT_VMCNT(0); else CTAMD_WAIT_VMCNT(LOADS * (S - 2));
+            if constexpr (Cfg::ABL == 3) c1 = __builtin_readcyclecounter();
+            __builtin_amdgcn_s_barrier();
+            if constexpr (Cfg::ABL == 3) { c2 = __builtin_readcyclecounter(); waitV += c1 - c0; waitB += c2 - c1; }
+            if constexpr (Cfg::ABL != 1) issue(slot);
+            slot = (slot + 1 == S) ? 0 : slot + 1;
+        }
+        if constexpr (Cfg::ABL == 3) {
+            if (tlog != nullptr && tid == 256) { tlog[9] = waitV; tlog[10] = waitB; }
+        }
+        for (; t + 1 < nTiles; ++t) {
+            const int behind = nTiles - t - 2;
+            if (behind <= 0) { CTAMD_WAIT_VMCNT(0); fix_last(); }
+            else if (behind == 1) CTAMD_WAIT_VMCNT(LOADS);
+            else if (behind == 2) CTAMD_WAIT_VMCNT(LOADS * 2);
+            else if (behind == 3) CTAMD_WAIT_VMCNT((S > 4 ? LOADS * 3 : 0));
+            else CTAMD_WAIT_VMCNT((S > 5 ? LOADS * 4 : 0));
+            __builtin_amdgcn_s_barrier();
+        }
+        CTAMD_WAIT_VMCNT(0);
+        return;
diff --git a/cudalibrarysamples_amd/csrc/kernels/launch.h b/cudalibrarysamples_amd/csrc/kernels/launch.h
--- a/cudalibrarysamples_amd/csrc/kernels/launch.h
+++ b/cudalibrarysamples_amd/csrc/kernels/launch.h
@@ -1,5 +1,7 @@
 #pragma once
 #include <hip/hip_runtime_api.h>
+
+#include <atomic>
 
 #include "params.h"
 
@@ -53,6 +55,7 @@
 hipError_t launch_splitk_reduce(const SplitKReduceParams& p, hipStream_t stream);
 hipError_t launch_splitk_reduce_frag(const SplitKReduceParams& p, hipStream_t stream);
 const GettKernelInfo* gett_f32_stream_kernels(int* count);
+extern std::atomic<uint64_t> g_flatStartLaunches;
 
 const GettKernelInfo* gett_h16_kernels(int* count);
 const GettKernelInfo* gett_h16v_kernels(int* count);
diff --git a/cudalibrarysamples_amd/csrc/kernels/params.h b/cudalibrarysamples_amd/csrc/kernels/params.h
--- a/cudalibrarysamples_amd/csrc/kernels/params.h
+++ b/cudalibrarysamples_amd/csrc/kernels/params.h
@@ -44,7 +44,24 @@
     uint32_t    ragged;
     uint32_t    mOrg, nOrg;
     uint32_t    tilesM2, tilesN2, mOrg2, nOrg2;
+    int32_t     noFlatStart;
 };
+
+struct StreamFlatParams {
+    const float* A;
+    const float* B;
+    float*       partial;
+    unsigned long long* timing;
+    uint32_t     sM, sN;
+    uint32_t     Mtot, Ntot;
+    uint32_t     splitK, kPerSlice, nBlocks;
+    uint32_t     kTotal;
+    uint32_t     kExt[kMaxGroupModes];
+    uint32_t     kMagic[kMaxGroupModes - 1];
+    uint32_t     kShifts;
+    uint32_t     kStrideA[kMaxGroupModes], kStrideB[kMaxGroupModes];
+};
+static_assert(sizeof(StreamFlatParams) == 128, "the flat entry's arguments are two 64-byte lines");
 
 struct WideMode {
     FastDiv div;
@@ -80,6 +97,7 @@
     int32_t      outType;
     double       alpha64, beta64, alphaIm, betaIm;
     int32_t      conjC;
+    int32_t      noFlatStart;
 };
 
 struct Ew2DParams {
diff --git a/cudalibrarysamples_amd/cutensor.py b/cudalibrarysamples_amd/cutensor.py
--- a/cudalibrarysamples_amd/cutensor.py
+++ b/cudalibrarysamples_amd/cutensor.py
@@ -101,6 +101,8 @@
 lib.ctamdPlanMemoStats.restype = None
 lib.ctamdLaunchCounts.argtypes = [ctypes.POINTER(ctypes.c_uint64)]
 lib.ctamdLaunchCounts.restype = None
+lib.ctamdFlatStartCount.argtypes = []
+lib.ctamdFlatStartCount.restype = ctypes.c_uint64
 lib.ctamdLastH16Kernel.argtypes = []
 lib.ctamdLastH16Kernel.restype = ctypes.c_int
 lib.ctamdSetTimingBuffer.argtypes = [_vp, _vp]
@@ -144,6 +146,10 @@
     return dict(zip(("simple", "wide", "f32", "h16", "gen"), [int(v) for v in out]))
 
 
+def flat_start_count():
+    return int(lib.ctamdFlatStartCount())
+
+
 def last_h16_kernel():
     return int(lib.ctamdLastH16Kernel())
 
```
